# schreibfaul1/ESP32-Opus-Player

Hardware: AMD Instinct MI355X
Metric: decoded 48 kHz stereo frames/sec/GPU (x real-time); HBM GB/s vs roofline (higher is better)
Workload: dtype int32 fixed-point (int16/int32 with 64-bit products); 1 GPU; celt_fb_stereo_64k; streams_per_gpu=65536

## Files before the change

### __graft_entry__.py

```python
import importlib.util
import os
import subprocess
import sys

ROOT = os.path.dirname(os.path.abspath(__file__))
PKG_DIR = os.path.join(ROOT, "esp32-opus-player_amd")
CSRC = os.path.join(PKG_DIR, "csrc")


def _load_pkg():
    name = "esp32_opus_player_amd"
    if name in sys.modules:
        return sys.modules[name]
    path = os.path.join(PKG_DIR, "__init__.py")
    spec = importlib.util.spec_from_file_location(name, path, submodule_search_locations=[PKG_DIR])
    mod = importlib.util.module_from_spec(spec)
    sys.modules[name] = mod
    spec.loader.exec_module(mod)
    return mod


def build() -> None:
    subprocess.check_call([sys.executable, os.path.join(ROOT, "tools", "gen_rom_tables.py")])
    hipcc = os.environ.get("HIPCC", "/opt/rocm/bin/hipcc")
    out = os.path.join(PKG_DIR, "libopusgpu.so")
    cmd = [hipcc, "--offload-arch=gfx950", "-O3", "-std=c++17", "-fPIC", "-shared",
           os.path.join(CSRC, "og_api.hip"), os.path.join(CSRC, "og_recon.hip"), os.path.join(CSRC, "og_parse64.hip"), os.path.join(CSRC, "og_rfc.hip"), os.path.join(CSRC, "og_silk_nb.hip"), os.path.join(CSRC, "og_silk_synth.hip"), os.path.join(CSRC, "og_compat.cpp"),
           os.path.join(CSRC, "og_pages.cpp"), os.path.join(CSRC, "og_files.cpp"),
           "-I", os.path.join(ROOT, "include"), "-pthread",
           "-o", out]
    cmd = [c for c in cmd if not c.endswith("og_compat.cpp") or os.path.exists(c)]
    flags_file = os.path.join(CSRC, "BUILD_FLAGS")
    if os.path.exists(flags_file):
        cmd += open(flags_file).read().split()
    subprocess.check_call(cmd)
    subprocess.check_call(["make", "-C", os.path.join(ROOT, "oracle"), "-s"])
    emul = os.path.join(ROOT, "tests", "emul")
    if os.path.exists(os.path.join(emul, "Makefile")):
        subprocess.check_call(["make", "-C", emul, "-s"])
    pkg = _load_pkg()
    lib = pkg.load_lib()
    missing = [s for s in pkg.EXPORTS if not hasattr(lib, s)]
    if missing:
        raise RuntimeError(f"libopusgpu.so lacks exports: {missing}")


def smoke() -> None:
    import numpy as np
    sys.path.insert(0, os.path.join(ROOT, "tests"))
    import oracle_py
    pkg = _load_pkg()
    oracle = oracle_py.load()
    ctx = pkg.Context(0)
    n, frames = 64, 3
    for name, toc, L in (("CELT-FB", pkg.TOC_CELT_FB_STEREO, 160), ("SILK-NB", pkg.TOC_SILK_NB_STEREO, 40),
                         ("hybrid FB", pkg.TOC_HYBRID_FB_STEREO, 120)):
        pay = pkg.lcg_payloads(n, frames, L)
        ref, ok = oracle.batch_decode(2, toc, pay)
        assert ok == n * frames
        ctx.streams_alloc(n, 2)
        for f in range(frames):
            pk = [bytes([toc]) + pay[f, s].tobytes() for s in range(n)]
            pcm, res = ctx.decode_packets(np.arange(n), pk)
            assert (res == 960).all(), (name, res)
            assert (pcm == ref[:, f]).all(), f"{name}: GPU PCM differs from the oracle"
    ctx.close()
    print("smoke ok: 64 streams x 3 frames x {CELT-FB, SILK-NB, hybrid FB} bit-exact vs oracle")


if __name__ == "__main__":
    build()
    if len(sys.argv) > 1 and sys.argv[1] == "smoke":
        smoke()
```

### esp32-opus-player_amd/csrc/og_api.hip

```cpp
#include <hip/hip_runtime.h>
#include <stdio.h>
#include <stdlib.h>
#include <string.h>
#include <condition_variable>
#include <functional>
#include <memory>
#include <new>
#include <mutex>
#include <thread>
#include <vector>
#include "og_decode.hpp"
#include "og_host_framing.hpp"
#include "og_output.hpp"
#include "og_debug.hpp"

using namespace og;

static_assert(sizeof(opusgpu_frame_desc) == sizeof(FrameDesc), "descriptor layout");

#define OG_STALL_MAX_SPINS (1 << 20)
__global__ void __launch_bounds__(64) k_stream_stall(long long ticks, int max_spins) {
    const long long t0 = wall_clock64();
    for (int i = 0; i < max_spins && wall_clock64() - t0 < ticks; i++) __builtin_amdgcn_s_sleep(8);
}
__global__ void __launch_bounds__(64) k_stream_init(StreamState *st, int first, int count, int channels, int full) {
    const int s = first + (int)blockIdx.x;
    if ((int)blockIdx.x >= count) return;
    if (full)
        stream_init(&st[s], channels);
    else
        stream_reset(&st[s]);
}

enum {
    CRC_CHUNK = 64,
    CRC_DEPTH = 1,
    CRC_LPL = CRC_CHUNK / 16,
    CRC_PPI = 64 / CRC_LPL,
    CRC_NL = 64 / CRC_PPI,
    CRC_ROW = CRC_CHUNK / 4 + 1,
    CRC_STEPS = CRC_CHUNK / 8
};
__global__ void __launch_bounds__(256) k_pages_crc(const u8 *__restrict__ blob, const long long *__restrict__ offs,
                                                    const i32 *__restrict__ lens, i32 *__restrict__ status, int n,
                                                    const u32 *__restrict__ tables) {
    __shared__ u32 T[8][256];
    __shared__ u32 tile[4][64 * CRC_ROW];
    __shared__ long long pg_start[4][64];
    __shared__ i32 pg_meta[4][64];
    for (int i = (int)threadIdx.x; i < 8 * 256; i += 256) T[i >> 8][i & 255] = tables[i];
    const int wv = (int)threadIdx.x >> 6, lane = (int)threadIdx.x & 63;
    const int p = (int)blockIdx.x * 256 + (int)threadIdx.x;
    int total = 0, st = OPUSGPU_PAGE_BAD_CAPTURE;
    u32 want = 0;
    long long at0 = 0;
    if (p < n) {
        const u8 *pg = blob + offs[p];
        const int len = lens[p];
        if (len >= 27) {
            u32 h[8];
            if (len >= 32) {
                const uint4 a = *reinterpret_cast<const uint4 *>(pg), b = *reinterpret_cast<const uint4 *>(pg + 16);
                h[0] = a.x; h[1] = a.y; h[2] = a.z; h[3] = a.w; h[4] = b.x; h[5] = b.y; h[6] = b.z; h[7] = b.w;
            } else {
                for (int i = 0; i < 8; i++) h[i] = 0;
                for (int i = 0; i < 27; i++) h[i >> 2] |= (u32)pg[i] << (8 * (i & 3));
            }
            const int nseg = (int)(h[6] >> 16) & 255, hdr = 27 + nseg;
            if (h[0] == 0x5367674fu  && (h[1] & 255u) == 0 && len >= hdr) {
                u32 body = 0;
                for (int i = 0; i < nseg; i += 16) {
                    u32 v[4];
                    if (27 + i + 16 <= len) {
                        const uint4 q = *reinterpret_cast<const uint4 *>(pg + 27 + i);
                        v[0] = q.x; v[1] = q.y; v[2] = q.z; v[3] = q.w;
                    } else {
                        v[0] = v[1] = v[2] = v[3] = 0;
                        for (int b = 0; b < 16 && i + b < nseg; b++) v[b >> 2] |= (u32)pg[27 + i + b] << (8 * (b & 3));
                    }
                    const int keep = nseg - i;
#pragma unroll
                    for (int d = 0; d < 4; d++) {
                        const int kd = keep - 4 * d;
                        const u32 m = kd >= 4 ? 0xffffffffu : kd <= 0 ? 0u : (1u << (8 * kd)) - 1u;
                        body = __builtin_amdgcn_sad_u8(v[d] & m, 0u, body);
                    }
                }
                if (len >= hdr + (int)body) {
                    total = hdr + (int)body;
                    st = 0;
                    want = h[5] >> 16 | h[6] << 16;
                }
            }
        }
        at0 = offs[p];
    }
    const int z = st < 0 ? 0 : (int)((reinterpret_cast<unsigned long long>(blob) + (unsigned long long)at0) & (unsigned long long)(CRC_CHUNK - 1));
    const int nfull = (z + total) / CRC_CHUNK, tail = (z + total) % CRC_CHUNK, chunks = nfull + (tail != 0);
    pg_start[wv][lane] = at0 - z;
    pg_meta[wv][lane] = z | total << 8;
    __syncthreads();
    int max_chunks = chunks;
    for (int d = 32; d; d >>= 1) max_chunks = max(max_chunks, __shfl_xor(max_chunks, d, 64));
    u32 crc = 0;
    const int grp = lane / CRC_LPL, quarter = lane % CRC_LPL;
    auto fetch = [&](int k, u32 (&w)[CRC_NL][4]) {
#pragma unroll
        for (int i = 0; i < CRC_NL; i++) {
            const int q = CRC_PPI * i + grp;
            const i32 meta = pg_meta[wv][q];
            const int idx = CRC_CHUNK * k + 16 * quarter - (meta & 255);
            w[i][0] = w[i][1] = w[i][2] = w[i][3] = 0u;
            if (idx > -16 && idx < (meta >> 8)) {
                const uint4 v = *reinterpret_cast<const uint4 *>(
                    __builtin_assume_aligned(blob + (pg_start[wv][q] + CRC_CHUNK * k + 16 * quarter), 16));
                w[i][0] = v.x; w[i][1] = v.y; w[i][2] = v.z; w[i][3] = v.w;
                if (idx < 26) {
#pragma unroll
                    for (int d = 0; d < 4; d++) {
                        u32 m = 0;
#pragma unroll
                        for (int c = 0; c < 4; c++) {
                            const int ib = idx + 4 * d + c;
                            if (ib >= 0 && !(ib >= 22 && ib <= 25)) m |= 0xffu << (8 * c);
                        }
                        w[i][d] &= m;
                    }
                }
            }
        }
    };
    auto consume = [&](int k, u32 (&w)[CRC_NL][4]) {
#pragma unroll
        for (int i = 0; i < CRC_NL; i++) {
            u32 *dst = &tile[wv][(CRC_PPI * i + grp) * CRC_ROW + 4 * quarter];
            dst[0] = w[i][0]; dst[1] = w[i][1]; dst[2] = w[i][2]; dst[3] = w[i][3];
        }
        __builtin_amdgcn_fence(__ATOMIC_RELEASE, "wavefront");
        __builtin_amdgcn_wave_barrier();
        __builtin_amdgcn_fence(__ATOMIC_ACQUIRE, "wavefront");
        if (k + CRC_DEPTH < max_chunks) fetch(k + CRC_DEPTH, w);
        const u32 *rowp = &tile[wv][lane * CRC_ROW];
        const int steps = k < nfull ? CRC_STEPS : k == nfull ? tail >> 3 : 0;
#pragma unroll
        for (int j = 0; j < CRC_STEPS; j++) {
            if (j < steps) {
                const u32 lo = rowp[2 * j], hi = rowp[2 * j + 1];
                const u32 a = crc ^ ((lo & 0xffu) << 24 | (lo & 0xff00u) << 8 | (lo >> 8 & 0xff00u) | lo >> 24);
                crc = T[7][a >> 24] ^ T[6][(a >> 16) & 255] ^ T[5][(a >> 8) & 255] ^ T[4][a & 255] ^ T[3][hi & 255] ^
                      T[2][(hi >> 8) & 255] ^ T[1][(hi >> 16) & 255] ^ T[0][hi >> 24];
            }
        }
        if (k == nfull && (tail & 7)) {
            const int base = tail & ~7;
            for (int b = 0; b < (tail & 7); b++) {
                const int i = base + b;
                crc = crc << 8 ^ T[0][crc >> 24 ^ (rowp[i >> 2] >> (8 * (i & 3)) & 255u)];
            }
        }
        __builtin_amdgcn_fence(__ATOMIC_RELEASE, "wavefront");
        __builtin_amdgcn_wave_barrier();
        __builtin_amdgcn_fence(__ATOMIC_ACQUIRE, "wavefront");
    };
    u32 wa[CRC_NL][4], wb[CRC_NL][4];
    if (max_chunks > 0) fetch(0, wa);
    if (CRC_DEPTH == 2) {
        if (max_chunks > 1) fetch(1, wb);
        for (int k = 0; k < max_chunks; k += 2) {
            consume(k, wa);
            if (k + 1 < max_chunks) consume(k + 1, wb);
        }
    } else {
        for (int k = 0; k < max_chunks; k++) consume(k, wa);
    }
    if (p < n) status[p] = st < 0 ? st : (i32)(crc == want);
}

static_assert(sizeof(opusgpu_output_cfg) == sizeof(OutputCfg) && sizeof(OutputCfg) == 4, "output cfg layout");
__global__ void __launch_bounds__(256) k_output_stage(const i16 *__restrict__ pcm, long long pcm_stride, const i32 *__restrict__ valid_of,
                                                       int valid_all, int block_samples, const OutputCfg *__restrict__ cfg_of,
                                                       OutputCfg cfg_all, u32 *__restrict__ out, long long out_stride,
                                                       int units_per_block, long long n_units, int vec_ok) {
    const long long t = (long long)blockIdx.x * 256 + threadIdx.x;
    if (t >= n_units) return;
    const int b = (int)(t / units_per_block), w0 = 4 * (int)(t - (long long)b * units_per_block);
    const OutputCfg c = cfg_of ? cfg_of[b] : cfg_all;
    int valid = valid_of ? valid_of[b] : valid_all;
    valid = valid > block_samples ? block_samples : valid;
    const int count = output_words(c, valid);
    if (w0 >= count) return;
    const i16 *blk = pcm + (size_t)b * pcm_stride;
    u32 *dst = out + (size_t)b * out_stride + w0;
    if (vec_ok && c.bits == 16 && c.channels == 2 && w0 + 4 <= count) {
        const uint4 v = *reinterpret_cast<const uint4 *>(blk + 2 * w0);
        const u32 in[4] = {v.x, v.y, v.z, v.w};
        u32 o[4];
#pragma unroll
        for (int j = 0; j < 4; j++) {
            i32 l = (i32)(i16)(in[j] & 0xffffu), r = (i32)(i16)(in[j] >> 16);
            if (c.force_mono) l = r = (i32)(i16)((l + r) / 2);
            o[j] = output_pack(l, r, false, (i32)c.volume);
        }
        *reinterpret_cast<uint4 *>(dst) = make_uint4(o[0], o[1], o[2], o[3]);
    } else {
        for (int j = 0; j < 4 && w0 + j < count; j++) dst[j] = output_word(blk, w0 + j, c);
    }
}

#ifndef OG_WAVES_PER_SIMD
#define OG_WAVES_PER_SIMD 1
#endif
#define OG_RECON_WAVES 2
#define OG_SILK_WAVES 2
__global__ void __launch_bounds__(64, OG_WAVES_PER_SIMD) k_decode_step(const FrameDesc *__restrict__ descs, const u8 *__restrict__ arena,
                                                   StreamState *st, i16 *pcm, i32 *result, int n, int n_streams,
                                                   int pcm_stride, int skip_celt, SilkHandoff *handoff, const SilkRec *srecs,
                                                   int q4_only) {
    unsigned long long todo = 1ull;
    int base = (int)blockIdx.x;
    if (q4_only) {
        base = (int)blockIdx.x * 64;
        const int f0 = base + (int)threadIdx.x;
        bool mine = false;
        if (f0 < n) {
            const FrameDesc d0 = descs[f0];
            mine = d0.stream >= 0 && d0.stream < n_streams && !desc_rfc(d0.flags) && desc_mode(d0.flags) == MODE_SILK && handoff[f0].valid == 2;
        }
        todo = __ballot(mine);
    }
    while (todo) {
        const int f = base + (int)__builtin_ctzll(todo);
        todo &= todo - 1;
        if (f >= n) return;
        const FrameDesc d = descs[f];
        int ret;
        if (d.stream < 0 || d.stream >= n_streams) {
            ret = BAD_ARG;
        } else if (desc_rfc(d.flags)) {
            continue;
        } else if (skip_celt && desc_mode(d.flags) == MODE_CELT) {
            continue;
        } else {
            StreamState *s = &st[d.stream];
#ifdef OG_PROF_SINGLE
            OG_PROF_INIT();
#endif
            ret = decode_frame_wave<true>(s, arena + d.offset, d.len, desc_mode(d.flags), desc_bandwidth(d.flags),
                                          desc_channels(d.flags), pcm + (size_t)f * pcm_stride, handoff ? &handoff[f] : nullptr,
                                          srecs ? &srecs[f] : nullptr, q4_only, desc_mode_after(d.flags));
#ifdef OG_PROF_SINGLE
            OG_PROF_FLUSH();
#endif
            if (ret == CONTINUE_SPLIT) continue;
        }
        if (threadIdx.x == 0) result[f] = ret;
        __syncthreads();
    }
}

extern "C" void og_launch_silk_synth(hipStream_t s, const void *descs, const void *arena, void *streams, void *pcm, void *result, int n,
                                     int n_streams, int pcm_stride, void *handoff, const void *srecs, int nb_elsewhere);
extern "C" void og_launch_silk_synth_nb(hipStream_t s, const void *descs, const void *arena, void *streams, void *pcm, void *result, int n,
                                        int n_streams, int pcm_stride, void *handoff, const void *srecs, int nb_elsewhere);

#define OG_SPARSE_WAVES 4
template <int LANES>
OG_DEV void silk_parse_kernel_body(const FrameDesc *__restrict__ descs, const u8 *__restrict__ arena, const StreamState *st, SilkRec *srecs,
                                   SilkHandoff *handoff, int n, int n_streams, SilkShadow *shadow, u32 epoch) {
    silk_tables_load();
    if ((int)threadIdx.x >= LANES) return;
    const int f = (int)blockIdx.x * LANES + (int)threadIdx.x;
    if (f >= n) return;
    const FrameDesc d = descs[f];
    const int mode = desc_mode(d.flags);
    if (d.stream < 0 || d.stream >= n_streams || mode == MODE_CELT || desc_rfc(d.flags)) return;
#ifdef OG_PROF_SPARSE
    OG_PROF_INIT();
#endif
    SilkShadow *const sh = shadow ? &shadow[d.stream] : nullptr;
    const SilkPast past(&st[d.stream], sh, epoch);
    silk_parse_lane(past, arena + d.offset, d.len, mode, desc_bandwidth(d.flags), desc_channels(d.flags), &srecs[f], &handoff[f], sh, epoch,
                    desc_mode_after(d.flags));
#ifdef OG_PROF_SPARSE
    OG_PROF_FLUSH();
#endif
}
__global__ void __launch_bounds__(64, OG_SPARSE_WAVES) k_silk_parse(const FrameDesc *__restrict__ descs, const u8 *__restrict__ arena,
                                                      const StreamState *st, SilkRec *srecs, SilkHandoff *handoff, int n,
                                                      int n_streams, SilkShadow *shadow, u32 epoch) {
    silk_parse_kernel_body<32>(descs, arena, st, srecs, handoff, n, n_streams, shadow, epoch);
}
__global__ void __launch_bounds__(64, OG_SPARSE_WAVES) k_silk_parse64(const FrameDesc *__restrict__ descs, const u8 *__restrict__ arena,
                                                        const StreamState *st, SilkRec *srecs, SilkHandoff *handoff, int n,
                                                        int n_streams, SilkShadow *shadow, u32 epoch) {
    silk_parse_kernel_body<64>(descs, arena, st, srecs, handoff, n, n_streams, shadow, epoch);
}

#define OG_SPARAMS_WAVES 4
__global__ void __launch_bounds__(64, OG_SPARAMS_WAVES) k_silk_params(const FrameDesc *__restrict__ descs, const StreamState *st, SilkRec *srecs,
                                                                       int n, int n_streams, SilkShadow *shadow, u32 epoch) {
    constexpr int FR = OG_PAR_LANES / 2;
    const int ch = (int)threadIdx.x / FR, f = (int)blockIdx.x * FR + (int)threadIdx.x % FR;
    bool act = f < n;
    FrameDesc d = {0, 0, 0, 0};
    if (act) {
        d = descs[f];
        act = !(d.stream < 0 || d.stream >= n_streams || desc_mode(d.flags) == MODE_CELT || desc_rfc(d.flags));
    }
    SilkShadow *const sh = act && shadow ? &shadow[d.stream] : nullptr;
    const SilkParPast past(act ? &st[d.stream] : st, sh, epoch);
    const int mode = desc_mode(d.flags), channels = desc_channels(d.flags);
    SilkParTask t;
    t.skip = 1;
    if (act) silk_params_channel(past, mode, desc_bandwidth(d.flags), channels, &srecs[f], ch, t);
    OG_FULL_SYNC();
    if (act) silk_params_shadow(past, t, channels, &srecs[f], ch, sh, epoch);
}

#define OG_PARSE_KERNEL_NAME k_celt_parse
#include "og_parse_kernel.hpp"
extern "C" void og_launch_celt_parse64(hipStream_t s, int grid, const void *descs, const void *arena, void *streams, void *recs, int n,
                                       int n_streams, const void *handoff, int which, int groups, unsigned *started);
extern "C" int og_celt_parse64_frames(void);

extern "C" void og_launch_celt_recon_fb(hipStream_t s, const void *descs, void *streams, const void *recs, void *rout, int n,
                                        int n_streams, int hybrid, unsigned *started);
extern "C" int og_celt_recon_fb_signals(int n);
extern "C" void og_launch_decode_rfc(hipStream_t s, const void *descs, const void *arena, void *streams, void *pcm, void *result, int n,
                                     int n_streams, int pcm_stride);
__global__ void __launch_bounds__(64, OG_RECON_WAVES) k_celt_recon(const FrameDesc *__restrict__ descs, StreamState *st,
                                                                      const ParseRec *recs, ReconOut *rout, int n,
                                                                      int n_streams, int hybrid, int rest_only) {
    unsigned long long todo = 1ull;
    int base = (int)blockIdx.x;
    if (rest_only) {
        base = (int)blockIdx.x * 64;
        const int f0 = base + (int)threadIdx.x;
        bool mine = false;
        if (f0 < n) {
            const FrameDesc d0 = descs[f0];
            const int m0 = desc_mode(d0.flags);
            if (d0.stream >= 0 && d0.stream < n_streams && (m0 == MODE_CELT || (m0 == MODE_HYBRID && hybrid)) && !desc_rfc(d0.flags)) {
                const u32 fl = recs[f0].flags;
                const bool fast = !(fl & (RF_SKIP | RF_BAD_CELT)) && ((fl >> RF_LM_SHIFT) & 3) == 3 && recs[f0].n_words < REC_MAX_WORDS &&
                                  recs[f0].n_leaves <= FAST_MAX_LEAVES;
                mine = !fast && !(m0 == MODE_HYBRID && (fl & RF_SKIP));
            }
        }
        todo = __ballot(mine);
    }
    while (todo) {
        const int f = base + (int)__builtin_ctzll(todo);
        todo &= todo - 1;
        if (f >= n) return;
        const FrameDesc d = descs[f];
        const int mode = desc_mode(d.flags);
        if (d.stream < 0 || d.stream >= n_streams || !(mode == MODE_CELT || (mode == MODE_HYBRID && hybrid)) || desc_rfc(d.flags)) continue;
        if (mode == MODE_HYBRID && (recs[f].flags & RF_SKIP)) continue;
#if !defined(OG_PROF_PARSE) && !defined(OG_PROF_SINGLE) && !defined(OG_PROF_SPARSE) && !defined(OG_PROF_SSYNTH)
        OG_PROF_INIT();
#endif
        const int pos = OG_UNI(st[d.stream].celt.ring_pos);
        const int ret = celt_recon_wave(&st[d.stream], &recs[f], mode, desc_channels(d.flags), rest_only ? RECON_REST_ONLY : RECON_ALL, desc_mode_after(d.flags));
        if (ret != RECON_NOT_MINE && threadIdx.x == 0) rout[f] = ReconOut{ret, pos};
#if !defined(OG_PROF_PARSE) && !defined(OG_PROF_SINGLE) && !defined(OG_PROF_SPARSE) && !defined(OG_PROF_SSYNTH)
        OG_PROF_FLUSH();
#endif
        __syncthreads();
    }
}

static __device__ __forceinline__ i32 pk_add_sat_i16(i32 a, i32 b) {
    typedef short s2 __attribute__((ext_vector_type(2)));
    const s2 r = __builtin_elementwise_add_sat(__builtin_bit_cast(s2, a), __builtin_bit_cast(s2, b));
    return __builtin_bit_cast(i32, r);
}
__global__ void __launch_bounds__(64) k_celt_post(const FrameDesc *__restrict__ descs, StreamState *st, const ParseRec *recs,
                                                  const ReconOut *__restrict__ rout, i32 *__restrict__ result, i16 *pcm, int n,
                                                  int n_streams, int channels, int pcm_stride, const SilkHandoff *handoff,
                                                  int modes, int others_ran) {
    struct RowInfo {
        const i32 *ring;
        i16 *pcm;
        const i16 *silk;
        int pos, silk_n;
    };
    constexpr int CS = 32, PCS = CS / 4, RSTEP = 64 / PCS;
    __shared__ RowInfo rows[64];
    __shared__ __attribute__((aligned(16))) i32 tin[64][CS + 4];
    __shared__ __attribute__((aligned(16))) i16 tout[64][CS + 8];
    const int lane = (int)threadIdx.x;
    const int t = (int)blockIdx.x * 64 + lane;
    const int f = channels == 2 ? t >> 1 : t, c = channels == 2 ? t & 1 : 0;
    bool live = false, emit = false;
    StreamState *ss = nullptr;
    const i16 *silk = nullptr;
    int silk_n = 0;
    int pos = 0;
    if (f < n) {
        const FrameDesc d = descs[f];
        const int mode = desc_mode(d.flags);
        const bool stream_ok = d.stream >= 0 && d.stream < n_streams;
        if (!(modes >> (d.flags & 3) & 1) || (!stream_ok && !others_ran)) {
            if (c == 0) result[f] = BAD_ARG;
        } else if (stream_ok && (mode == MODE_CELT || (mode == MODE_HYBRID && handoff)) && !desc_rfc(d.flags)) {
            const u32 rf = recs[f].flags;
            if (!(mode == MODE_HYBRID && (rf & RF_SKIP))) {
                const ReconOut ro = rout[f];
                if (c == 0) result[f] = ro.ret;
                if (!(rf & (RF_SKIP | RF_BAD_CELT))) {
                    live = true;
                    ss = &st[d.stream];
                    emit = ro.ret >= 0;
                    pos = ro.pos & RING_MASK;
                    if (mode == MODE_HYBRID) {
                        silk = handoff[f].pcm;
                        silk_n = 960 * desc_channels(d.flags);
                    }
                }
            }
        }
    }
    i16 *out = pcm + (size_t)(f < n ? f : 0) * pcm_stride;
    const bool fast = channels == 2 && __all(live && emit && (pos & (CS - 1)) == 0);
    if (!fast) {
        if (live) celt_post_lane(&ss->celt, c, channels, 960, pos, emit ? out : nullptr, silk, silk_n);
        return;
    }
    rows[lane].ring = ss->celt.ring[c];
    rows[lane].pcm = out;
    rows[lane].silk = silk;
    rows[lane].pos = pos;
    rows[lane].silk_n = silk_n;
    __syncthreads();
    const int q = lane % PCS, r0 = lane / PCS;
    const i32 *src[PCS];
    int spos[PCS];
#pragma unroll
    for (int k = 0; k < PCS; k++) {
        src[k] = rows[r0 + RSTEP * k].ring;
        spos[k] = rows[r0 + RSTEP * k].pos + 4 * q;
    }
    og_v4i v[PCS];
#pragma unroll
    for (int k = 0; k < PCS; k++) v[k] = *reinterpret_cast<const og_v4i *>(src[k] + (spos[k] & RING_MASK));
    i32 m = ss->celt.deemph[c];
    for (int ch = 0; ch < 960 / CS; ch++) {
#pragma unroll
        for (int k = 0; k < PCS; k++) *reinterpret_cast<og_v4i *>(&tin[r0 + RSTEP * k][4 * q]) = v[k];
        if (ch + 1 < 960 / CS) {
#pragma unroll
            for (int k = 0; k < PCS; k++) v[k] = *reinterpret_cast<const og_v4i *>(src[k] + ((spos[k] + CS * (ch + 1)) & RING_MASK));
        }
        __syncthreads();
#pragma unroll
        for (int g8 = 0; g8 < CS / 8; g8++) {
            i16 o[8];
#pragma unroll
            for (int h = 0; h < 2; h++) {
                const og_v4i sv = *reinterpret_cast<const og_v4i *>(&tin[lane][8 * g8 + 4 * h]);
                i32 tt = sv.x + m;
                m = mul16x32_q15(27853, tt);
                o[4 * h + 0] = (i16)sat16(pshr32(tt, 12));
                tt = sv.y + m;
                m = mul16x32_q15(27853, tt);
                o[4 * h + 1] = (i16)sat16(pshr32(tt, 12));
                tt = sv.z + m;
                m = mul16x32_q15(27853, tt);
                o[4 * h + 2] = (i16)sat16(pshr32(tt, 12));
                tt = sv.w + m;
                m = mul16x32_q15(27853, tt);
                o[4 * h + 3] = (i16)sat16(pshr32(tt, 12));
            }
            og_v4i w;
            w.x = (i32)((u32)(u16)o[0] | (u32)(u16)o[1] << 16);
            w.y = (i32)((u32)(u16)o[2] | (u32)(u16)o[3] << 16);
            w.z = (i32)((u32)(u16)o[4] | (u32)(u16)o[5] << 16);
            w.w = (i32)((u32)(u16)o[6] | (u32)(u16)o[7] << 16);
            *reinterpret_cast<og_v4i *>(&tout[lane][8 * g8]) = w;
        }
        __syncthreads();
#pragma unroll
        for (int k = 0; k < PCS / 2; k++) {
            const int fr = r0 + RSTEP * k;
            const og_v2u L = *reinterpret_cast<const og_v2u *>(&tout[2 * fr][4 * q]);
            const og_v2u R = *reinterpret_cast<const og_v2u *>(&tout[2 * fr + 1][4 * q]);
            og_v4i w;
            w.x = (i32)((L.x & 0xffffu) | R.x << 16);
            w.y = (i32)(L.x >> 16 | (R.x & 0xffff0000u));
            w.z = (i32)((L.y & 0xffffu) | R.y << 16);
            w.w = (i32)(L.y >> 16 | (R.y & 0xffff0000u));
            const int at = (CS * ch + 4 * q) * 2;
            const i16 *const sk = rows[2 * fr].silk;
            if (sk && at < rows[2 * fr].silk_n) {
                const og_v4i a = *reinterpret_cast<const og_v4i *>(sk + at);
                w.x = pk_add_sat_i16(w.x, a.x);
                w.y = pk_add_sat_i16(w.y, a.y);
                w.z = pk_add_sat_i16(w.z, a.z);
                w.w = pk_add_sat_i16(w.w, a.w);
            }
            *reinterpret_cast<og_v4i *>(rows[2 * fr].pcm + at) = w;
        }
    }
    ss->celt.deemph[c] = m;
}

#include "og_step.hpp"

const size_t og_parse_rec_bytes = sizeof(ParseRec), og_recon_out_bytes = sizeof(ReconOut), og_silk_handoff_bytes = sizeof(SilkHandoff),
             og_silk_rec_bytes = sizeof(SilkRec);
namespace {
struct StepRange {
    const FrameDesc *dd;
    i16 *pp;
    i32 *rr;
    ParseRec *recs;
    ReconOut *rout;
    SilkHandoff *hh;
    SilkRec *srecs;
    StepRange(const Step &st, size_t f0)
        : dd((const FrameDesc *)st.descs + f0), pp((i16 *)st.pcm + f0 * (size_t)st.pcm_stride), rr((i32 *)st.result + f0),
          recs((ParseRec *)st.recs + f0), rout((ReconOut *)st.rout + f0), hh(st.handoff ? (SilkHandoff *)st.handoff + f0 : nullptr),
          srecs(st.srecs ? (SilkRec *)st.srecs + f0 : nullptr) {}
};
}
void launch_stream_stall(opusgpu_ctx *ctx, hipStream_t q) {
    hipLaunchKernelGGL(k_stream_stall, dim3(1), dim3(64), 0, q, ctx->stall_ticks, (int)OG_STALL_MAX_SPINS);
}
void launch_decode_rfc(opusgpu_ctx *ctx, hipStream_t q, const Step &st) {
    og_launch_decode_rfc(q, st.descs, st.arena, ctx->d_streams, st.pcm, st.result, st.n, ctx->n_streams, st.pcm_stride);
}
void launch_decode_step(opusgpu_ctx *ctx, hipStream_t q, const Step &st, size_t f0, int cnt, int pass) {
    const StepRange r(st, f0);
    hipLaunchKernelGGL(k_decode_step, dim3(pass == 2 ? (cnt + 63) / 64 : cnt), dim3(64), 0, q, r.dd, (const u8 *)st.arena, ctx->d_streams, r.pp,
                       r.rr, cnt, ctx->n_streams, st.pcm_stride, pass ? 1 : 0, pass == 2 ? r.hh : nullptr,
                       (const SilkRec *)(pass == 2 ? r.srecs : nullptr), pass == 2 ? 1 : 0);
}
void launch_silk_parse(opusgpu_ctx *ctx, hipStream_t q, const Step &st, size_t f0, int cnt, void *shadow, uint32_t epoch) {
    const StepRange r(st, f0);
    hipLaunchKernelGGL(k_silk_parse, dim3((cnt + 31) / 32), dim3(64), 0, q, r.dd, (const u8 *)st.arena, (const StreamState *)ctx->d_streams,
                       r.srecs, r.hh, cnt, ctx->n_streams, (SilkShadow *)shadow, epoch);
}
void launch_silk_parse64(opusgpu_ctx *ctx, hipStream_t q, const Step &st, size_t f0, int cnt, void *shadow, uint32_t epoch) {
    const StepRange r(st, f0);
    hipLaunchKernelGGL(k_silk_parse64, dim3((cnt + 63) / 64), dim3(64), 0, q, r.dd, (const u8 *)st.arena, (const StreamState *)ctx->d_streams,
                       r.srecs, r.hh, cnt, ctx->n_streams, (SilkShadow *)shadow, epoch);
}
void launch_silk_params(opusgpu_ctx *ctx, hipStream_t q, const Step &st, size_t f0, int cnt, void *shadow, uint32_t epoch) {
    const StepRange r(st, f0);
    hipLaunchKernelGGL(k_silk_params, dim3((cnt + OG_PAR_LANES / 2 - 1) / (OG_PAR_LANES / 2)), dim3(64), 0, q, r.dd,
                       (const StreamState *)ctx->d_streams, r.srecs, cnt, ctx->n_streams, (SilkShadow *)shadow, epoch);
}
int celt_parse_early_grid(const opusgpu_ctx *ctx, int cnt, bool wide) {
    const int per = (wide ? og_celt_parse64_frames() : OG_PL_FRAMES) * ctx->parse_groups;
    return (cnt + per - 1) / per;
}
void launch_celt_parse(opusgpu_ctx *ctx, hipStream_t q, const Step &st, size_t f0, int cnt, bool wide, bool early) {
    const StepRange r(st, f0);
    const int which = early ? (int)PARSE_CELT_ONLY : (int)PARSE_ALL, groups = early ? ctx->parse_groups : 1;
    const int per = wide ? og_celt_parse64_frames() : OG_PL_FRAMES;
    const int grid = early ? celt_parse_early_grid(ctx, cnt, wide) : (cnt + per - 1) / per;
    u32 *const started = early ? ctx->sp.d_started : nullptr;
    if (wide)
        og_launch_celt_parse64(q, grid, r.dd, st.arena, ctx->d_streams, r.recs, cnt, ctx->n_streams, r.hh, which, groups, started);
    else
        hipLaunchKernelGGL(k_celt_parse, dim3(grid), dim3(64 * OG_PL_WAVES), 0, q, r.dd, (const u8 *)st.arena, ctx->d_streams, r.recs, cnt,
                           ctx->n_streams, (const SilkHandoff *)r.hh, which, groups, started);
}
void launch_celt_recon_fb(opusgpu_ctx *ctx, hipStream_t q, const Step &st, size_t f0, int cnt, bool counts_in) {
    const StepRange r(st, f0);
    og_launch_celt_recon_fb(q, r.dd, ctx->d_streams, r.recs, r.rout, cnt, ctx->n_streams, r.hh ? 1 : 0, counts_in ? ctx->sp.d_started + 16 : nullptr);
}
void launch_celt_recon(opusgpu_ctx *ctx, hipStream_t q, const Step &st, size_t f0, int cnt) {
    const StepRange r(st, f0);
    hipLaunchKernelGGL(k_celt_recon, dim3(ctx->fast_recon ? (cnt + 63) / 64 : cnt), dim3(64), 0, q, r.dd, ctx->d_streams, (const ParseRec *)r.recs,
                       r.rout, cnt, ctx->n_streams, r.hh ? 1 : 0, ctx->fast_recon);
}
void launch_celt_post(opusgpu_ctx *ctx, hipStream_t q, const Step &st, size_t f0, int cnt, bool others) {
    const StepRange r(st, f0);
    hipLaunchKernelGGL(k_celt_post, dim3((cnt * ctx->channels + 63) / 64), dim3(64), 0, q, r.dd, ctx->d_streams, (const ParseRec *)r.recs,
                       (const ReconOut *)r.rout, r.rr, r.pp, cnt, ctx->n_streams, ctx->channels, st.pcm_stride, (const SilkHandoff *)r.hh, st.modes,
                       others ? 1 : 0);
}
void launch_silk_synth(opusgpu_ctx *ctx, hipStream_t q, const Step &st, size_t f0, int cnt, int nb_done) {
    const StepRange r(st, f0);
    og_launch_silk_synth(q, r.dd, st.arena, ctx->d_streams, r.pp, r.rr, cnt, ctx->n_streams, st.pcm_stride, r.hh, r.srecs, nb_done);
}
void launch_silk_synth_nb(opusgpu_ctx *ctx, hipStream_t q, const Step &st, size_t f0, int cnt) {
    const StepRange r(st, f0);
    og_launch_silk_synth_nb(q, r.dd, st.arena, ctx->d_streams, r.pp, r.rr, cnt, ctx->n_streams, st.pcm_stride, r.hh, r.srecs, 1);
}


extern "C" {


int opusgpu_version(void) { return 100; }

int opusgpu_ctx_create(int device, opusgpu_ctx **out) {
    if (!out || device < 0) return OPUSGPU_BAD_ARG;
    *out = nullptr;
    int count = 0;
    if (hipGetDeviceCount(&count) != hipSuccess || count <= 0 || device >= count) return OPUSGPU_ERR_NO_DEVICE;
    if (hipSetDevice(device) != hipSuccess) return OPUSGPU_ERR_NO_DEVICE;
    hipFuncAttributes attr;
    if (hipFuncGetAttributes(&attr, reinterpret_cast<const void *>(k_decode_step)) != hipSuccess) {
        (void)hipGetLastError();
        return OPUSGPU_ERR_NO_DEVICE;
    }
    opusgpu_ctx *ctx = new (std::nothrow) opusgpu_ctx();
    if (!ctx) return OPUSGPU_ALLOC_FAIL;
    ctx->device = device;
    ctx->split_celt = og_debug().split;
    ctx->split_hybrid = og_debug().split_hybrid;
    ctx->fast_recon = og_debug().fast_recon;
    ctx->parse_groups = og_debug().parse_groups;
    ctx->host_parts = og_debug().host_parts;
    if (og_debug().stall_us) {
        int khz = 0;
        if (hipDeviceGetAttribute(&khz, hipDeviceAttributeWallClockRate, device) != hipSuccess || khz <= 0) {
            (void)hipGetLastError();
            delete ctx;
            return OPUSGPU_ERR_HIP;
        }
        ctx->stall_ticks = (long long)og_debug().stall_us * khz / 1000;
    }
    if (hipStreamCreateWithFlags(&ctx->stream, hipStreamNonBlocking) != hipSuccess) {
        delete ctx;
        return OPUSGPU_ERR_HIP;
    }
    *out = ctx;
    return OPUSGPU_OK;
}

void opusgpu_ctx_destroy(opusgpu_ctx *ctx) {
    if (!ctx) return;
    (void)hipSetDevice(ctx->device);
    (void)hipStreamSynchronize(ctx->stream);
    (void)hipFree(ctx->d_streams);
    (void)hipFree(ctx->d_descs);
    (void)hipFree(ctx->d_arena);
    (void)hipFree(ctx->d_pcm);
    (void)hipFree(ctx->d_result);
    pipeline_destroy(ctx);
    for (int i = 0; i < 6; i++) {
        (void)hipFree(ctx->d_recs[i]);
        (void)hipFree(ctx->d_rout[i]);
    }
    for (int i = 0; i < OG_SILK_SETS; i++) {
        (void)hipFree(ctx->d_handoff[i]);
        (void)hipFree(ctx->d_srecs[i]);
    }
    (void)hipFree(ctx->d_shadow);
    (void)hipHostFree(ctx->h_pcm);
    (void)hipHostFree(ctx->h_res);
    (void)hipHostFree(ctx->h_arena);
    (void)hipHostFree(ctx->h_descs);
    (void)hipFree(ctx->d_crc_tables);
    for (hipEvent_t e : ctx->ev_piece)
        if (e) (void)hipEventDestroy(e);
    for (hipEvent_t e : ctx->ev_part)
        if (e) (void)hipEventDestroy(e);
    if (ctx->copy_stream) (void)hipStreamDestroy(ctx->copy_stream);
    (void)hipStreamDestroy(ctx->stream);
    delete ctx;
}

const char *opusgpu_last_error(const opusgpu_ctx *ctx) { return ctx ? ctx->err : "no context"; }
int opusgpu_set_mode(opusgpu_ctx *ctx, int mode) {
    if (!ctx || (mode != OPUSGPU_MODE_REFERENCE && mode != OPUSGPU_MODE_RFC)) return OPUSGPU_BAD_ARG;
    ctx->mode = mode;
    return OPUSGPU_OK;
}
int opusgpu_get_mode(const opusgpu_ctx *ctx) { return ctx ? ctx->mode : OPUSGPU_MODE_REFERENCE; }
int opusgpu_set_pipeline(opusgpu_ctx *ctx, int on) {
    if (!ctx) return OPUSGPU_BAD_ARG;
    HIPCHK(ctx, hipSetDevice(ctx->device));
    if (on)
        if (int rc = pipeline_create(ctx)) return rc;
    if ((on != 0) != (ctx->pipeline != 0)) {
        HIPCHK(ctx, hipDeviceSynchronize());
        ctx->sp.drained();
        ctx->sp.last_kind = 0;
        ctx->sp.shadow_epoch++;
    }
    ctx->pipeline = on ? 1 : 0;
    return OPUSGPU_OK;
}
int opusgpu_get_pipeline(const opusgpu_ctx *ctx) { return ctx ? ctx->pipeline : 0; }
size_t opusgpu_stream_state_bytes(void) { return sizeof(StreamState); }
int opusgpu_stream_count(const opusgpu_ctx *ctx) { return ctx ? ctx->n_streams : 0; }
int opusgpu_stream_channels(const opusgpu_ctx *ctx) { return ctx ? ctx->channels : 0; }

int opusgpu_streams_reset(opusgpu_ctx *ctx, int first, int count, int full) {
    if (!ctx || first < 0 || count < 0 || first + count > ctx->n_streams) return OPUSGPU_BAD_ARG;
    if (count == 0) return OPUSGPU_OK;
    HIPCHK(ctx, hipSetDevice(ctx->device));
    if (int rc = sync_in_flight(ctx)) return rc;
    ctx->sp.drained();
    ctx->sp.shadow_epoch++;
    hipLaunchKernelGGL(k_stream_init, dim3(count), dim3(64), 0, ctx->stream, ctx->d_streams, first, count, ctx->channels,
                       full ? 1 : 0);
    HIPCHK(ctx, hipGetLastError());
    HIPCHK(ctx, hipStreamSynchronize(ctx->stream));
    for (int i = first; i < first + count; i++) ctx->last_count[i] = ctx->last_flags[i] = 0;
    return OPUSGPU_OK;
}

int opusgpu_streams_alloc(opusgpu_ctx *ctx, int n_streams, int channels) {
    if (!ctx || n_streams <= 0 || (channels != 1 && channels != 2)) return OPUSGPU_BAD_ARG;
    HIPCHK(ctx, hipSetDevice(ctx->device));
    HIPCHK(ctx, hipStreamSynchronize(ctx->stream));
    if (int rc = sync_in_flight(ctx)) return rc;
    if (ctx->d_streams) {
        HIPCHK(ctx, hipFree(ctx->d_streams));
        ctx->d_streams = nullptr;
        ctx->n_streams = 0;
    }
    hipError_t e = hipMalloc((void **)&ctx->d_streams, sizeof(StreamState) * (size_t)n_streams);
    if (e != hipSuccess) return fail(ctx, OPUSGPU_ALLOC_FAIL, "hipMalloc(streams)", e);
    if (ctx->d_shadow) HIPCHK(ctx, hipFree(ctx->d_shadow));
    ctx->d_shadow = nullptr;
    e = hipMalloc(&ctx->d_shadow, sizeof(SilkShadow) * (size_t)n_streams);
    if (e != hipSuccess) return fail(ctx, OPUSGPU_ALLOC_FAIL, "hipMalloc(shadow)", e);
    HIPCHK(ctx, hipMemset(ctx->d_shadow, 0, sizeof(SilkShadow) * (size_t)n_streams));
    ctx->sp.shadow_epoch++;
    ctx->n_streams = n_streams;
    ctx->channels = channels;
    ctx->last_count.assign((size_t)n_streams, 0);
    ctx->last_flags.assign((size_t)n_streams, 0);
    return opusgpu_streams_reset(ctx, 0, n_streams, 1);
}

int opusgpu_dev_alloc(opusgpu_ctx *ctx, size_t bytes, void **dptr) {
    if (!ctx || !dptr) return OPUSGPU_BAD_ARG;
    HIPCHK(ctx, hipSetDevice(ctx->device));
    if (bytes > SIZE_MAX - 16) return OPUSGPU_ALLOC_FAIL;
    hipError_t e = hipMalloc(dptr, bytes + 16);
    if (e != hipSuccess) return fail(ctx, OPUSGPU_ALLOC_FAIL, "hipMalloc", e);
    return OPUSGPU_OK;
}
int opusgpu_dev_free(opusgpu_ctx *ctx, void *dptr) {
    if (!ctx) return OPUSGPU_BAD_ARG;
    HIPCHK(ctx, hipSetDevice(ctx->device));
    HIPCHK(ctx, hipFree(dptr));
    return OPUSGPU_OK;
}
int opusgpu_memcpy_h2d(opusgpu_ctx *ctx, void *dst, const void *src, size_t bytes) {
    if (!ctx) return OPUSGPU_BAD_ARG;
    HIPCHK(ctx, hipSetDevice(ctx->device));
    HIPCHK(ctx, hipMemcpyAsync(dst, src, bytes, hipMemcpyHostToDevice, ctx->stream));
    HIPCHK(ctx, hipStreamSynchronize(ctx->stream));
    return OPUSGPU_OK;
}
int opusgpu_memcpy_d2h(opusgpu_ctx *ctx, void *dst, const void *src, size_t bytes) {
    if (!ctx) return OPUSGPU_BAD_ARG;
    HIPCHK(ctx, hipSetDevice(ctx->device));
    if (int rc = sync_in_flight(ctx)) return rc;
    HIPCHK(ctx, hipMemcpyAsync(dst, src, bytes, hipMemcpyDeviceToHost, ctx->stream));
    HIPCHK(ctx, hipStreamSynchronize(ctx->stream));
    return OPUSGPU_OK;
}


int opusgpu_decode_step_device(opusgpu_ctx *ctx, int n, const void *d_descs, const void *d_arena, void *d_pcm,
                               void *d_result, void *hip_stream) {
    return decode_step_impl(ctx, n, d_descs, d_arena, d_pcm, d_result, hip_stream, true);
}
int opusgpu_decode_step_device_modes(opusgpu_ctx *ctx, int n, const void *d_descs, const void *d_arena, void *d_pcm,
                                     void *d_result, void *hip_stream, int modes) {
    if (modes <= 0 || modes > 15 || (modes & 7) == 0) return OPUSGPU_BAD_ARG;
    return decode_step_impl(ctx, n, d_descs, d_arena, d_pcm, d_result, hip_stream, true, modes);
}
int opusgpu_decode_steps_device(opusgpu_ctx *ctx, int n_steps, const int32_t *n, const void *const *d_descs, const void *const *d_arena,
                                void *const *d_pcm, void *const *d_result, void *hip_stream, int modes) {
    if (!ctx || n_steps < 0 || modes < 0 || modes > 7) return OPUSGPU_BAD_ARG;
    if (n_steps == 0) return OPUSGPU_OK;
    if (!n || !d_descs || !d_arena || !d_pcm || !d_result) return OPUSGPU_BAD_ARG;
    if (!ctx->d_streams) return OPUSGPU_BAD_ARG;
    int max_n = 0;
    for (int k = 0; k < n_steps; k++) {
        if (n[k] < 0) return OPUSGPU_BAD_ARG;
        if (n[k] > 0 && (!d_descs[k] || !d_arena[k] || ((uintptr_t)d_arena[k] & 15) || !d_pcm[k] || !d_result[k])) return OPUSGPU_BAD_ARG;
        max_n = OG_MAX(max_n, n[k]);
    }
    if (max_n == 0) return OPUSGPU_OK;
    return decode_window(ctx, n_steps, n, max_n, d_descs, d_arena, d_pcm, d_result, hip_stream, modes ? modes : 7);
}

#ifdef OG_PROF
extern "C" int og_recon_fb_prof(unsigned long long *out64, int reset);
extern "C" int og_rfc_prof(unsigned long long *out64, int reset);
extern "C" int og_ssynth_prof(unsigned long long *out64, int reset);
extern "C" int og_ssynth_nb_prof(unsigned long long *out64, int reset);
int opusgpu_debug_prof(unsigned long long *out64, int reset) {
    unsigned long long fb[64], rf[64];
    if (og_recon_fb_prof(fb, reset) != 0 || og_rfc_prof(rf, reset) != 0) return -1;
    for (int i = 0; i < 64; i++) fb[i] += rf[i];
    if (og_ssynth_prof(rf, reset) != 0) return -1;
    for (int i = 0; i < 64; i++) fb[i] += rf[i];
    if (og_ssynth_nb_prof(rf, reset) != 0) return -1;
    for (int i = 0; i < 64; i++) fb[i] += rf[i];
    if (hipMemcpyFromSymbol(out64, HIP_SYMBOL(g_prof), sizeof(unsigned long long) * 64) != hipSuccess) return -1;
    for (int i = 0; i < 64; i++) out64[i] += fb[i];
    if (reset) {
        unsigned long long z[64] = {0};
        if (hipMemcpyToSymbol(HIP_SYMBOL(g_prof), z, sizeof(z)) != hipSuccess) return -1;
    }
    return 0;
}
#endif

int opusgpu_pages_crc_device(opusgpu_ctx *ctx, int n_pages, const void *d_blob, const void *d_offsets, const void *d_lens,
                             void *d_status, void *hip_stream) {
    if (!ctx || n_pages < 0) return OPUSGPU_BAD_ARG;
    if (n_pages == 0) return OPUSGPU_OK;
    if (!d_blob || !d_offsets || !d_lens || !d_status) return OPUSGPU_BAD_ARG;
    HIPCHK(ctx, hipSetDevice(ctx->device));
    hipStream_t s = hip_stream ? (hipStream_t)hip_stream : ctx->stream;
    if (!ctx->d_crc_tables) {
        static u32 t[8][256];
        for (u32 i = 0; i < 256; i++) {
            u32 r = i << 24;
            for (int k = 0; k < 8; k++) r = (r & 0x80000000u) ? (r << 1) ^ 0x04c11db7u : r << 1;
            t[0][i] = r;
        }
        for (int j = 1; j < 8; j++)
            for (u32 i = 0; i < 256; i++) t[j][i] = (t[j - 1][i] << 8) ^ t[0][t[j - 1][i] >> 24];
        if (hipMalloc((void **)&ctx->d_crc_tables, sizeof(t)) != hipSuccess) return OPUSGPU_ALLOC_FAIL;
        HIPCHK(ctx, hipMemcpy(ctx->d_crc_tables, t, sizeof(t), hipMemcpyHostToDevice));
    }
    hipLaunchKernelGGL(k_pages_crc, dim3((n_pages + 255) / 256), dim3(256), 0, s, (const u8 *)d_blob, (const long long *)d_offsets,
                       (const i32 *)d_lens, (i32 *)d_status, n_pages, (const u32 *)ctx->d_crc_tables);
    HIPCHK(ctx, hipGetLastError());
    return OPUSGPU_OK;
}

int opusgpu_output_stage_device(opusgpu_ctx *ctx, int n_blocks, int block_samples, const void *d_pcm, long long pcm_stride,
                                const void *d_valid, int valid_all, const void *d_cfgs, opusgpu_output_cfg cfg, void *d_i2s,
                                long long i2s_stride, void *hip_stream) {
    if (!ctx || n_blocks < 0 || block_samples < 0) return OPUSGPU_BAD_ARG;
    if (n_blocks == 0 || block_samples == 0) return OPUSGPU_OK;
    if (!d_pcm || !d_i2s || pcm_stride < 0 || i2s_stride < 0) return OPUSGPU_BAD_ARG;
    if (!d_valid && (valid_all < 0 || valid_all > block_samples)) return OPUSGPU_BAD_ARG;
    if (!d_cfgs && ((cfg.bits != 8 && cfg.bits != 16) || (cfg.channels != 1 && cfg.channels != 2))) return OPUSGPU_BAD_ARG;
    HIPCHK(ctx, hipSetDevice(ctx->device));
    hipStream_t s = hip_stream ? (hipStream_t)hip_stream : ctx->stream;
    const int max_words = (d_cfgs || (cfg.bits == 8 && cfg.channels == 1)) ? 2 * block_samples : block_samples;
    const int units = (max_words + 3) / 4;
    const long long n_units = (long long)units * n_blocks;
    const int vec_ok = ((uintptr_t)d_pcm % 16 == 0 && pcm_stride % 8 == 0 && (uintptr_t)d_i2s % 16 == 0 && i2s_stride % 4 == 0) ? 1 : 0;
    OutputCfg c;
    memcpy(&c, &cfg, sizeof c);
    hipLaunchKernelGGL(k_output_stage, dim3((unsigned)((n_units + 255) / 256)), dim3(256), 0, s, (const i16 *)d_pcm, pcm_stride,
                       (const i32 *)d_valid, valid_all, block_samples, (const OutputCfg *)d_cfgs, c, (u32 *)d_i2s, i2s_stride, units,
                       n_units, vec_ok);
    HIPCHK(ctx, hipGetLastError());
    return OPUSGPU_OK;
}

int opusgpu_synchronize(opusgpu_ctx *ctx) {
    if (!ctx) return OPUSGPU_BAD_ARG;
    HIPCHK(ctx, hipStreamSynchronize(ctx->stream));
    return OPUSGPU_OK;
}

int opusgpu_event_create(opusgpu_ctx *ctx, void **event) {
    if (!ctx || !event) return OPUSGPU_BAD_ARG;
    hipEvent_t e;
    HIPCHK(ctx, hipEventCreate(&e));
    *event = (void *)e;
    return OPUSGPU_OK;
}
int opusgpu_event_record(opusgpu_ctx *ctx, void *event) {
    if (!ctx || !event) return OPUSGPU_BAD_ARG;
    HIPCHK(ctx, hipEventRecord((hipEvent_t)event, ctx->stream));
    return OPUSGPU_OK;
}
int opusgpu_event_elapsed_ms(opusgpu_ctx *ctx, void *start, void *stop, float *ms) {
    if (!ctx || !start || !stop || !ms) return OPUSGPU_BAD_ARG;
    HIPCHK(ctx, hipEventSynchronize((hipEvent_t)stop));
    HIPCHK(ctx, hipEventElapsedTime(ms, (hipEvent_t)start, (hipEvent_t)stop));
    return OPUSGPU_OK;
}
int opusgpu_event_destroy(opusgpu_ctx *ctx, void *event) {
    if (!ctx || !event) return OPUSGPU_BAD_ARG;
    HIPCHK(ctx, hipEventDestroy((hipEvent_t)event));
    return OPUSGPU_OK;
}

static std::mutex g_copy_stream_mutex;
static int copy_stream_of(opusgpu_ctx *ctx, hipStream_t *out) {
    std::lock_guard<std::mutex> lock(g_copy_stream_mutex);
    if (!ctx->copy_stream) HIPCHK(ctx, hipStreamCreateWithFlags(&ctx->copy_stream, hipStreamNonBlocking));
    *out = ctx->copy_stream;
    return OPUSGPU_OK;
}
int opusgpu_upload_async(opusgpu_ctx *ctx, void *dst, const void *src, size_t bytes) {
    if (!ctx || (bytes && (!dst || !src))) return OPUSGPU_BAD_ARG;
    HIPCHK(ctx, hipSetDevice(ctx->device));
    hipStream_t cs;
    if (int rc = copy_stream_of(ctx, &cs)) return rc;
    if (bytes) HIPCHK(ctx, hipMemcpyAsync(dst, src, bytes, hipMemcpyHostToDevice, cs));
    return OPUSGPU_OK;
}
int opusgpu_upload_fence(opusgpu_ctx *ctx, void *event) {
    if (!ctx || !event) return OPUSGPU_BAD_ARG;
    HIPCHK(ctx, hipSetDevice(ctx->device));
    hipStream_t cs;
    if (int rc = copy_stream_of(ctx, &cs)) return rc;
    HIPCHK(ctx, hipEventRecord((hipEvent_t)event, cs));
    return OPUSGPU_OK;
}
int opusgpu_stream_wait_event(opusgpu_ctx *ctx, void *event, void *hip_stream) {
    if (!ctx || !event) return OPUSGPU_BAD_ARG;
    HIPCHK(ctx, hipSetDevice(ctx->device));
    HIPCHK(ctx, hipStreamWaitEvent(hip_stream ? (hipStream_t)hip_stream : ctx->stream, (hipEvent_t)event, 0));
    if ((!hip_stream || (hipStream_t)hip_stream == ctx->stream) && ctx->sp.parse_stream) {
        HIPCHK(ctx, hipStreamWaitEvent(ctx->sp.parse_stream, (hipEvent_t)event, 0));
        HIPCHK(ctx, hipStreamWaitEvent(ctx->sp.recon_stream, (hipEvent_t)event, 0));
    }
    return OPUSGPU_OK;
}
int opusgpu_event_synchronize(opusgpu_ctx *ctx, void *event) {
    if (!ctx || !event) return OPUSGPU_BAD_ARG;
    HIPCHK(ctx, hipSetDevice(ctx->device));
    HIPCHK(ctx, hipEventSynchronize((hipEvent_t)event));
    return OPUSGPU_OK;
}
int opusgpu_host_register(opusgpu_ctx *ctx, void *ptr, size_t bytes) {
    if (!ctx || !ptr || !bytes) return OPUSGPU_BAD_ARG;
    HIPCHK(ctx, hipSetDevice(ctx->device));
    hipError_t e = hipHostRegister(ptr, bytes, hipHostRegisterDefault);
    if (e != hipSuccess) return fail(ctx, OPUSGPU_ALLOC_FAIL, "hipHostRegister", e);
    std::lock_guard<std::mutex> lock(ctx->registered_mutex);
    ctx->registered.emplace_back((uintptr_t)ptr, bytes);
    return OPUSGPU_OK;
}
int opusgpu_host_unregister(opusgpu_ctx *ctx, void *ptr) {
    if (!ctx || !ptr) return OPUSGPU_BAD_ARG;
    HIPCHK(ctx, hipSetDevice(ctx->device));
    {
        std::lock_guard<std::mutex> lock(ctx->registered_mutex);
        for (size_t i = 0; i < ctx->registered.size(); i++)
            if (ctx->registered[i].first == (uintptr_t)ptr) {
                ctx->registered.erase(ctx->registered.begin() + i);
                break;
            }
    }
    HIPCHK(ctx, hipHostUnregister(ptr));
    return OPUSGPU_OK;
}

int opusgpu_stream_state_get(opusgpu_ctx *ctx, int index, void *dst, size_t bytes) {
    if (!ctx || !dst || index < 0 || index >= ctx->n_streams || bytes > sizeof(StreamState)) return OPUSGPU_BAD_ARG;
    return opusgpu_memcpy_d2h(ctx, dst, &ctx->d_streams[index], bytes);
}

int opusgpu_stream_pitch_get(opusgpu_ctx *ctx, int index, int32_t out[4]) {
    if (!ctx || !out || index < 0 || index >= ctx->n_streams) return OPUSGPU_BAD_ARG;
    int32_t head[2], ch0[3];
    if (int rc = opusgpu_memcpy_d2h(ctx, head, &ctx->d_streams[index], sizeof(head))) return rc;
    const SilkChannel *c = &ctx->d_streams[index].silk.ch[0];
    HIPCHK(ctx, hipMemcpy(&ch0[0], &c->prevSignalType, 4, hipMemcpyDeviceToHost));
    HIPCHK(ctx, hipMemcpy(&ch0[1], &c->lagPrev, 4, hipMemcpyDeviceToHost));
    HIPCHK(ctx, hipMemcpy(&ch0[2], &c->fs_kHz, 4, hipMemcpyDeviceToHost));
    out[0] = head[1];
    out[1] = ch0[0];
    out[2] = ch0[1];
    out[3] = ch0[2];
    return OPUSGPU_OK;
}

int opusgpu_debug_stage_taps(opusgpu_ctx *ctx, int slot, opusgpu_stage_taps *out) {
    if (!ctx || !out || slot < 0 || slot >= ctx->last_n || !ctx->last_descs) return OPUSGPU_BAD_ARG;
    HIPCHK(ctx, hipSetDevice(ctx->device));
    if (int rc = sync_in_flight(ctx)) return rc;
    HIPCHK(ctx, hipStreamSynchronize(ctx->stream));
    memset(out, 0, sizeof(*out));
    FrameDesc d;
    HIPCHK(ctx, hipMemcpy(&d, (const FrameDesc *)ctx->last_descs + slot, sizeof(d), hipMemcpyDeviceToHost));
    if (d.stream < 0 || d.stream >= ctx->n_streams) return OPUSGPU_BAD_ARG;
    const int mode = MODE_SILK + (d.flags & 3);
    std::unique_ptr<StreamState> st(new (std::nothrow) StreamState);
    if (!st) return OPUSGPU_ALLOC_FAIL;
    HIPCHK(ctx, hipMemcpy(st.get(), &ctx->d_streams[d.stream], sizeof(StreamState), hipMemcpyDeviceToHost));
    if (mode != MODE_SILK && ctx->last_recs) {
        std::unique_ptr<ParseRec> r(new (std::nothrow) ParseRec);
        if (!r) return OPUSGPU_ALLOC_FAIL;
        HIPCHK(ctx, hipMemcpy(r.get(), (const ParseRec *)ctx->last_recs + slot, sizeof(ParseRec), hipMemcpyDeviceToHost));
        out->celt_valid = 1;
        out->celt_ret = r->ret;
        out->silence = (r->flags & RF_SILENCE) != 0;
        out->transient = (r->flags & RF_TRANSIENT) != 0;
        out->lm = (int)(r->flags >> RF_LM_SHIFT) & 3;
        out->spread = (int)(r->flags >> RF_SPREAD_SHIFT) & 3;
        out->dual_stereo = (r->flags & RF_DUAL) != 0;
        out->anti_collapse_on = (r->flags & RF_ANTI_COLLAPSE) != 0;
        out->intensity = r->intensity;
        out->pf_pitch = r->pf_pitch;
        out->pf_gain = r->pf_gain;
        out->pf_tapset = r->pf_tapset;
        out->n_leaves = r->n_leaves;
        out->celt_rng_final = r->rng_final;
        memcpy(out->bandE, r->bandE, sizeof(out->bandE));
        memcpy(out->pulses, r->pulses, sizeof(out->pulses));
        memcpy(out->tf_res, r->tf_res, sizeof(out->tf_res));
    }
    const CeltState &c = st->celt;
    for (int ch = 0; ch < 2; ch++) {
        for (int i = 0; i < 960; i++) out->syn_post[ch][i] = c.ring[ch][(c.ring_pos - 960 + i) & RING_MASK];
        for (int i = 0; i < 60; i++) out->overlap_tail[ch][i] = c.tail[ch][i];
    }
    memcpy(out->state_bandE, c.bandE, sizeof(out->state_bandE));
    memcpy(out->state_logE1, c.logE1, sizeof(out->state_logE1));
    memcpy(out->state_logE2, c.logE2, sizeof(out->state_logE2));
    out->state_rng = c.rng;
    out->pf_period = c.pf_period;
    out->pf_gain_state = c.pf_gain;
    out->pf_tapset_state = c.pf_tapset;
    if (mode != MODE_CELT && ctx->last_had_silk_recs && ctx->last_srecs) {
        std::unique_ptr<SilkRec> r(new (std::nothrow) SilkRec);
        if (!r) return OPUSGPU_ALLOC_FAIL;
        HIPCHK(ctx, hipMemcpy(r.get(), (const SilkRec *)ctx->last_srecs + slot, sizeof(SilkRec), hipMemcpyDeviceToHost));
        out->silk_valid = 1;
        out->silk_ret = r->ret;
        out->decode_only_middle = r->decode_only_middle;
        out->ms_pred_q13[0] = r->MS_pred_Q13[0];
        out->ms_pred_q13[1] = r->MS_pred_Q13[1];
        for (int ch = 0; ch < 2; ch++) {
            const SilkRecCh &k = r->ch[ch];
            memcpy(out->silk_ch[ch].pitchL, k.pitchL, sizeof(k.pitchL));
            memcpy(out->silk_ch[ch].Gains_Q16, k.Gains_Q16, sizeof(k.Gains_Q16));
            memcpy(out->silk_ch[ch].PredCoef_Q12, k.PredCoef_Q12, sizeof(k.PredCoef_Q12));
            memcpy(out->silk_ch[ch].LTPCoef_Q14, k.LTPCoef_Q14, sizeof(k.LTPCoef_Q14));
            out->silk_ch[ch].LTP_scale_Q14 = k.LTP_scale_Q14;
            out->silk_ch[ch].signalType = k.signalType;
            out->silk_ch[ch].quantOffsetType = k.quantOffsetType;
        }
    }
    for (int ch = 0; ch < 2; ch++) {
        memcpy(out->silk_out[ch], st->silk.ch[ch].outBuf, sizeof(out->silk_out[ch]));
        memcpy(out->silk_sLPC_Q14[ch], st->silk.ch[ch].sLPC_Q14_buf, sizeof(out->silk_sLPC_Q14[ch]));
        out->silk_fs_kHz[ch] = st->silk.ch[ch].fs_kHz;
    }
    return OPUSGPU_OK;
}

int opusgpu_packet_to_frames(const uint8_t *packet, int32_t len, int32_t stream, opusgpu_frame_desc descs[48]) {
    return opusgpu_packet_to_frames_mode(packet, len, stream, OPUSGPU_MODE_REFERENCE, descs);
}

int opusgpu_packet_to_frames_mode(const uint8_t *packet, int32_t len, int32_t stream, int mode, opusgpu_frame_desc descs[48]) {
    if (!packet || !descs) return OPUSGPU_BAD_ARG;
    if (len <= 0) return len == 0 ? OPUSGPU_INVALID_PACKET : OPUSGPU_BAD_ARG;
    return ogh::packet_to_frames_mode(packet, len, stream, mode, descs);
}

int opusgpu_empty_packet_to_frames(int32_t stream, int32_t last_flags, int decoder_channels, int frame_size, opusgpu_frame_desc descs[48]) {
    if (!descs || frame_size <= 0 || frame_size % 120 || (decoder_channels != 1 && decoder_channels != 2)) return OPUSGPU_BAD_ARG;
    const int count = (frame_size + OPUSGPU_FRAME_SAMPLES - 1) / OPUSGPU_FRAME_SAMPLES;
    if (count > 48) return OPUSGPU_BAD_ARG;
    const int32_t flags = ogh::empty_flags(last_flags, decoder_channels);
    for (int i = 0; i < count; i++) descs[i] = opusgpu_frame_desc{stream, 0, 0, flags};
    return count;
}

static int grow(opusgpu_ctx *ctx, void **p, size_t *cap, size_t need) {
    if (*cap >= need) return OPUSGPU_OK;
    if (*p) HIPCHK(ctx, hipFree(*p));
    *p = nullptr;
    *cap = 0;
    size_t want = need + need / 2 + 256;
    hipError_t e = hipMalloc(p, want);
    if (e != hipSuccess) return fail(ctx, OPUSGPU_ALLOC_FAIL, "hipMalloc(staging)", e);
    *cap = want;
    return OPUSGPU_OK;
}

}

#include "og_host_path.hpp"

#include "og_ms.hpp"
#include "og_files_run.hpp"
#include "og_tracks.hpp"
#include "og_ms_tracks.hpp"
```

### esp32-opus-player_amd/csrc/og_celt_rec.hpp

```cpp
#pragma once
#include <stddef.h>
#include "og_state.hpp"

namespace og {

constexpr int REC_BAND_WORDS = 4;
constexpr int REC_MAX_LEAVES = NBANDS * 2 * 16;
constexpr int REC_MAX_WORDS = NBANDS * (REC_BAND_WORDS + 2 * 33) + 3 * NBANDS + 1;

enum {
    RF_SILENCE = 1, RF_TRANSIENT = 2, RF_LM_SHIFT = 2 , RF_STEREO = 16, RF_SPREAD_SHIFT = 5 ,
    RF_DUAL = 128, RF_ANTI_COLLAPSE = 256, RF_RC_ERROR = 512, RF_TELL_OVERFLOW = 1024,
    RF_SKIP = 2048,
    RF_BAD_CELT = 4096
};
enum {
    BW_SIGN0 = 1, BW_SIGN1 = 2, BW_INV = 4, BW_SIGN = 8, BW_MID_FIRST = 16, BW_SWAP = 32,
    BW_THETA0 = 64, BW_THETA1 = 128,
    BW_TF_SHIFT = 8 , BW_FOLD0_SHIFT = 11 , BW_FOLD1_SHIFT = 16 ,
    BW_HAS_LOW = 1 << 21, BW_DUAL = 1 << 22, BW_DUAL_END = 1 << 23, BW_STEREO = 1 << 24,
    BW_DUAL_PRE = 1 << 25
};
enum {
    JW_NPVQ_SHIFT = 5 , JW_FIRST_SHIFT = 10 , JW_NEED_LOW = 1 << 20,
    LW_OFF_SHIFT = 8 , LW_B_SHIFT = 12 , LW_N_SHIFT = 16
};

struct SilkHandoff {
    alignas(128) i16 pcm[1920];
    u32 valid;
    u32 storage, end_offs, end_window;
    i32 nend_bits, nbits_total;
    u32 offs, rng, val, ext;
    i32 rem, error;
};
static_assert(sizeof(SilkHandoff) % 128 == 0 && offsetof(SilkHandoff, pcm) == 0, "handoff alignment");

struct ParseRec {
    i32 ret;
    u32 rng_final;
    u32 flags;
    i32 intensity, pf_pitch, pf_gain, pf_tapset, start;
    i32 n_leaves, n_words;
    u32 need_norm;
    i32 n_coef;
    i32 reserved[4];
    i16 bandE[2 * NBANDS];
    i16 pulses[NBANDS];
    u16 band_w[NBANDS];
    i8 tf_res[NBANDS];
    i8 pad[256 - 64 - 4 * NBANDS - 2 * NBANDS - 2 * NBANDS - NBANDS];
    struct Leaf {
        u32 idx;
        u32 geom;
        u32 aux;
        u32 pad;
    } leaf[REC_MAX_LEAVES];
    u32 words[(REC_MAX_WORDS + 64) / 64 * 64];
    i32 work_pulses[NBANDS];
    i32 work_pad[32 - NBANDS];
};
static_assert(offsetof(ParseRec, leaf) % 16 == 0 && offsetof(ParseRec, words) % 16 == 0 && offsetof(ParseRec, work_pulses) % 16 == 0 &&
              offsetof(ParseRec, work_pad) == offsetof(ParseRec, work_pulses) + 4 * NBANDS && NBANDS + 3 <= 32, "16-byte stores into the record");
static_assert(sizeof(ParseRec) % 16 == 0, "record alignment");

constexpr int FAST_MAX_LEAVES = 416;

struct ReconOut {
    i32 ret, pos;
};

}
```

### esp32-opus-player_amd/csrc/og_celt_recon.hpp

```cpp
#pragma once
#include "og_celt.hpp"
#include "og_celt_rec.hpp"

namespace og {

#ifdef OG_HOST_EMUL
OG_DEV i32 rot_dot2(u32 pair, u32 coef, i32 half) {
    return (i32)((u32)mul16((i32)pair, (i32)coef) + (u32)mul16((i32)(pair >> 16), (i32)(coef >> 16)) + (u32)half) >> 15;
}
OG_DEV u32 rot_pack(i32 lo, i32 hi) { return ((u32)lo & 0xffffu) | (u32)hi << 16; }
#else
OG_DEV i32 rot_dot2(u32 pair, u32 coef, i32 half) {
    i32 r;
    asm("v_dot2_i32_i16 %0, %1, %2, %3" : "=v"(r) : "v"(pair), "v"(coef), "v"(half));
    return r >> 15;
}
OG_DEV u32 rot_pack(i32 lo, i32 hi) { return __builtin_amdgcn_perm((u32)hi, (u32)lo, 0x05040100u); }
#endif
OG_DEV void rotate_chain(i16 *const p0, int r, int len, int stride, u32 k_a, u32 k_b) {
    const i32 half = 16384;
    int i = r, steps = 0;
    i32 x1 = p0[i];
    for (; i + 3 * stride < len - stride; i += 4 * stride, steps += 4) {
        const i32 e1 = p0[i + stride], e2 = p0[i + 2 * stride], e3 = p0[i + 3 * stride], e4 = p0[i + 4 * stride];
        u32 pk = rot_pack(x1, e1);
        const i32 o0 = rot_dot2(pk, k_a, half);
        x1 = rot_dot2(pk, k_b, half);
        pk = rot_pack(x1, e2);
        const i32 o1 = rot_dot2(pk, k_a, half);
        x1 = rot_dot2(pk, k_b, half);
        pk = rot_pack(x1, e3);
        const i32 o2 = rot_dot2(pk, k_a, half);
        x1 = rot_dot2(pk, k_b, half);
        pk = rot_pack(x1, e4);
        const i32 o3 = rot_dot2(pk, k_a, half);
        x1 = rot_dot2(pk, k_b, half);
        p0[i] = (i16)o0;
        p0[i + stride] = (i16)o1;
        p0[i + 2 * stride] = (i16)o2;
        p0[i + 3 * stride] = (i16)o3;
    }
    for (; i < len - stride; i += stride, steps++) {
        const u32 pk = rot_pack(x1, p0[i + stride]);
        p0[i] = (i16)rot_dot2(pk, k_a, half);
        x1 = rot_dot2(pk, k_b, half);
    }
    p0[i] = (i16)x1;
    if (steps >= 2) {
        i -= 2 * stride;
        i32 x2 = p0[i + stride];
        for (; i - 3 * stride >= 0; i -= 4 * stride) {
            const i32 e1 = p0[i], e2 = p0[i - stride], e3 = p0[i - 2 * stride], e4 = p0[i - 3 * stride];
            u32 pk = rot_pack(e1, x2);
            const i32 o0 = rot_dot2(pk, k_b, half);
            x2 = rot_dot2(pk, k_a, half);
            pk = rot_pack(e2, x2);
            const i32 o1 = rot_dot2(pk, k_b, half);
            x2 = rot_dot2(pk, k_a, half);
            pk = rot_pack(e3, x2);
            const i32 o2 = rot_dot2(pk, k_b, half);
            x2 = rot_dot2(pk, k_a, half);
            pk = rot_pack(e4, x2);
            const i32 o3 = rot_dot2(pk, k_b, half);
            x2 = rot_dot2(pk, k_a, half);
            p0[i + stride] = (i16)o0;
            p0[i] = (i16)o1;
            p0[i - stride] = (i16)o2;
            p0[i - 2 * stride] = (i16)o3;
        }
        for (; i >= 0; i -= stride) {
            const u32 pk = rot_pack(p0[i], x2);
            p0[i + stride] = (i16)rot_dot2(pk, k_b, half);
            x2 = rot_dot2(pk, k_a, half);
        }
        p0[r] = (i16)x2;
    }
}
OG_DEV void rotate1_lane(i16 *xv, int x, int len, int stride, i32 c, i32 s) {
    const u32 k_a = rot_pack(c, -s), k_b = rot_pack(s, c);
    for (int r = 0; r < stride; r++) {
        if (r >= len - stride) break;
        rotate_chain(xv + x, r, len, stride, k_a, k_b);
    }
}

struct RotJob {
    int x, blen, logB, stride2;
    i32 c, s;
    bool on;
};
#ifndef OG_HOST_EMUL
OG_DEV void pvq_rotate_wave(i16 *xv, const RotJob &j, u8 *marker) {
    if (!__any(j.on)) return;
    const int lane = OG_LANE;
    const int w_geo = j.x | j.blen << 16, w_par = j.logB | j.stride2 << 8;
    const int w_cs = (int)((u32)(u16)j.c | (u32)(u16)j.s << 16);
    for (int pass = 0; pass < 2; pass++) {
        int chains = 0;
        if (j.on) chains = pass == 0 ? (j.stride2 ? OG_MAX(0, OG_MIN(j.stride2, j.blen - j.stride2)) : 0) : (j.blen >= 2);
        const int cnt = chains << j.logB;
        const int incl = wave_scan_add(cnt), excl = incl - cnt;
        const int total = __builtin_amdgcn_readlane(incl, 63);
        for (int base = 0; base < total; base += 64) {
            marker[lane] = 0;
            OG_LSYNC();
            if (cnt > 0 && excl < base + 64 && incl > base) marker[OG_MAX(excl - base, 0)] = (u8)(lane + 1);
            OG_LSYNC();
            const int leaf = wave_scan_max((int)marker[lane]) - 1;
            const int item = base + lane;
            const bool work = item < total;
            const int src = leaf < 0 ? lane : leaf;
            const int g = __shfl(w_geo, src), q = __shfl(w_par, src), cs = __shfl(w_cs, src), first = __shfl(excl, src);
            if (work) {
                const int logB = q & 255, sub = item - first, b = sub & ((1 << logB) - 1), r = sub >> logB;
                const int blen = g >> 16;
                const i32 c = (i32)(i16)(cs & 0xffff), sn = (i32)(i16)(cs >> 16);
                i16 *const p0 = xv + (g & 0xffff) + b * blen;
                const i32 cc = pass == 0 ? sn : c, ss = pass == 0 ? c : sn;
                rotate_chain(p0, r, blen, pass == 0 ? q >> 8 : 1, rot_pack(cc, -ss), rot_pack(ss, cc));
            }
            OG_LSYNC();
        }
    }
}
#endif

#ifdef OG_RECON_TIGHT
constexpr int PVQ_MAIN_LEN = ROM_PVQ_RB9, PVQ_TOP0_OFF = (X_TOP0 - V_NORM) / 2, PVQ_TOP1_OFF = (X_TOP1 - V_NORM) / 2;
static_assert((ROM_PVQ_RB12 - ROM_PVQ_RB9) * 2 <= 160 && (ROM_PVQ_RR_LEN - ROM_PVQ_RB12) * 2 + 32 <= 160, "the short rows (and the rotation marker) fit the tops");
#else
constexpr int PVQ_MAIN_LEN = ROM_PVQ_RR_LEN;
#endif
struct PvqLds {
    u32 rr[PVQ_MAIN_LEN];
    i16 rb[16];
    OG_MEMBER u32 at(int i) const { return reinterpret_cast<const u32 *>(this)[i]; }
};
OG_DEV int pvq_lds_index(int t) {
#ifdef OG_RECON_TIGHT
    return t < ROM_PVQ_RB9 ? t : t < ROM_PVQ_RB12 ? t - ROM_PVQ_RB9 + PVQ_TOP0_OFF : t - ROM_PVQ_RB12 + PVQ_TOP1_OFF;
#else
    return t;
#endif
}
#ifdef OG_RECON_TIGHT
static_assert(sizeof(PvqLds) <= (V_JOBM - V_NORM) * 2, "the PVQ table's long rows end before the jobs' collapse masks");
#else
static_assert(sizeof(PvqLds) <= (V_TOTAL - V_NORM) * 2, "the PVQ table overlays the folding-history, pulse and scratch rows");
#endif
OG_DEV PvqLds &pvq_lds() { return *reinterpret_cast<PvqLds *>(&S.v[V_NORM]); }
OG_DEV void pvq_tab_load() {
    u32 *const dst = reinterpret_cast<u32 *>(&pvq_lds());
#ifdef OG_HOST_EMUL
    OG_FOR_LANES(t, ROM_PVQ_RR_LEN) dst[pvq_lds_index(t)] = rom_pvq_rr[t];
    OG_FOR_LANES(t, 16) pvq_lds().rb[t] = (i16)pvq_lds_index(rom_pvq_rb[t]);
#else
    constexpr int NRR = (ROM_PVQ_RR_LEN + OG_NLANES - 1) / OG_NLANES;
    u32 rr[NRR];
#pragma unroll
    for (int k = 0; k < NRR; k++) rr[k] = rom_pvq_rr[OG_MIN(OG_LANE + k * OG_NLANES, ROM_PVQ_RR_LEN - 1)];
    const u16 rb = rom_pvq_rb[OG_LANE & 15];
#pragma unroll
    for (int k = 0; k < NRR; k++)
        if (OG_LANE + k * OG_NLANES < ROM_PVQ_RR_LEN) dst[pvq_lds_index(OG_LANE + k * OG_NLANES)] = rr[k];
    if (OG_LANE < 16) pvq_lds().rb[OG_LANE] = (i16)pvq_lds_index((int)rb);
#endif
}
OG_DEV u32 pvq_row_sel(int r, u32 v2, u32 v3) {
    u32 v = (u32)(r >= 1);
    v = r == 2 ? v2 : v;
    return r == 3 ? v3 : v;
}
#ifdef OG_HOST_EMUL
OG_DEV u32 pvq_u3(u32 h) { return 2u * h * (h - 1u) + 1u; }
OG_DEV int pvq_isqrt_near(u32 tq) { return (int)__builtin_sqrtf((float)tq); }
#else
OG_DEV u32 pvq_u3(u32 h) {
    u32 r;
    const u32 a = h << 1, b = h - 1u;
    asm("v_mad_u32_u24 %0, %1, %2, 1" : "=v"(r) : "v"(a), "v"(b));
    return r;
}
OG_DEV int pvq_isqrt_near(u32 tq) { return (int)__builtin_amdgcn_sqrtf((float)tq); }
#endif
#ifdef OG_HOST_EMUL
OG_DEV u32 pvq_block_mul(int blen) { return blen > 0 ? 65536u / (u32)blen + 1u : 0u; }
OG_DEV int pvq_block_of(int j, u32 mul) { return (int)(((u32)j * mul) >> 16); }
#else
OG_DEV u32 pvq_block_mul(int blen) { return (u32)(65536.0f * __builtin_amdgcn_rcpf((float)blen)) + 1u; }
OG_DEV int pvq_block_of(int j, u32 mul) { return (int)(__umul24((u32)j, mul) >> 16); }
#endif
OG_DEV int pvq_row_base(const PvqLds &T, int r) { return (int)T.rb[r < 4 ? 4 : (r > 14 ? 14 : r)]; }

OG_DEV u32 pvq_leaf_lane(i16 *xv, const PvqLds &T, int n, int k, u32 i, int pos, int B, i32 gain, int spread, RotJob *defer = nullptr) {
    const int N = n, K = k, x = pos;
    const int logB = ilog2(B), blen = N >> logB;
    i32 yy = 0;
    const u32 bmul = pvq_block_mul(blen);
    u32 cm = 0;
    OG_MARK(56);
    int b0 = pvq_row_base(T, k), b1 = pvq_row_base(T, k + 1);
    while (n > 2) {
        if (k == 0) break;
        u32 h = (u32)n, v2 = 2u * h - 1u, v3 = pvq_u3(h);
        const bool sparse = n > k;
        u32 p0, p1;
        int bn = 0;
        bool tab = false;
        if (sparse) {
            const u32 c0 = T.at(k >= 4 ? b0 + n : 0), c1 = T.at(k >= 3 ? b1 + n : 0);
            p0 = k >= 4 ? c0 : pvq_row_sel(k, v2, v3);
            p1 = k >= 3 ? c1 : pvq_row_sel(k + 1, v2, v3);
            if (k <= 13 && n > k && n > 3) {
                const u32 Vn = p0 + p1, t = Vn - i, m = i >= t ? i - t + 1u : t - i;
                const int lo0 = k + 1 > 2 ? k + 1 : 2;
                int a;
                u32 t0 = p0, t1 = p1;
                if (k <= 2) {
                    const u32 tq = (m + 1u) >> 1;
                    int r = (int)tq;
                    if (k == 2) {
                        r = pvq_isqrt_near(tq);
                        r += (u32)(r * r) < tq;
                    }
                    a = r > lo0 ? r : lo0;
                    const u32 u2 = 2u * (u32)a - 1u;
                    t0 = k == 1 ? 1u : u2;
                    t1 = k == 1 ? u2 : pvq_u3((u32)a);
                } else {
                    int lo = lo0, hi = n;
                    while (lo < hi) {
                        const int mid = (lo + hi) >> 1;
                        const u32 m0 = T.at(k >= 4 ? b0 + mid : 0), m1 = T.at(b1 + mid);
                        const u32 a0 = k >= 4 ? m0 : pvq_u3((u32)mid);
                        if (a0 + m1 >= m) {
                            hi = mid;
                            t0 = a0;
                            t1 = m1;
                        } else
                            lo = mid + 1;
                    }
                    a = lo;
                }
                if (a < n) {
                    i -= (Vn - (t0 + t1)) >> 1;
                    pos += n - a;
                    n = a;
                    if (n <= 2) break;
                    h = (u32)n;
                    v2 = 2u * h - 1u;
                    v3 = pvq_u3(h);
                    p0 = t0;
                    p1 = t1;
                }
            }
        } else {
            const u32 hk = (u32)k;
            bn = pvq_row_base(T, n);
            tab = n >= 4;
            const u32 a0 = T.at(tab ? bn + k : 0), a1 = T.at(tab ? bn + k + 1 : 0);
            p0 = tab ? a0 : pvq_u3(hk);
            p1 = tab ? a1 : pvq_u3(hk + 1u);
        }
        const int s = -(int)(i >= p1);
        i -= p1 & (u32)s;
        if (p0 <= i && s == 0) {
            i -= p0;
        } else {
            u32 plo = 0;
            const bool tabp = sparse || tab;
            const int off = sparse ? n : bn;
            int lo = sparse ? OG_MIN(3, k - 1) : 0, hi = k - 1;
            while (lo < hi) {
                const int mid = (lo + hi + 1) >> 1;
                const int rbm = pvq_row_base(T, mid);
                const u32 tm = T.at(tabp ? (sparse ? rbm : mid) + off : 0);
                const u32 pm = tabp ? tm : pvq_u3((u32)mid);
                if (pm <= i) {
                    lo = mid;
                    plo = pm;
                } else
                    hi = mid - 1;
            }
            int kk = lo;
            if (sparse && lo <= 3) {
                const u32 cand[3] = {1u, v2, v3};
                kk = 0;
#pragma unroll
                for (int r = 1; r <= 3; r++) {
                    const bool ok = r < k && cand[r - 1] <= i;
                    kk = ok ? r : kk;
                    plo = ok ? cand[r - 1] : plo;
                }
            }
            const int val = (k - kk + s) ^ s;
            k = kk;
            i -= plo;
            xv[pos] = (i16)val;
            cm |= 1u << pvq_block_of(pos - x, bmul);
            yy += val * val;
            b0 = pvq_row_base(T, k);
            b1 = pvq_row_base(T, k + 1);
        }
        pos++;
        n--;
    }
    {
        const u32 p = 2 * (u32)k + 1;
        int s = -(int)(i >= p);
        i -= p & (u32)s;
        const int k0 = k;
        k = (int)((i + 1) >> 1);
        if (k) i -= 2 * (u32)k - 1;
        int val = (k0 - k + s) ^ s;
        xv[pos] = (i16)val;
        cm |= (u32)(val != 0) << pvq_block_of(pos - x, bmul);
        pos++;
        yy += val * val;
        s = -(int)i;
        val = (k + s) ^ s;
        xv[pos] = (i16)val;
        cm |= (u32)(val != 0) << pvq_block_of(pos - x, bmul);
        yy += val * val;
    }
#ifdef OG_PVQ_WALK_TAP
    OG_PVQ_WALK_TAP(xv + x, N, yy);
#endif
    OG_MARK(57);
    cm = B > 1 ? cm & ((1u << B) - 1u) : 1u;
    OG_MARK(58);
    const int kk = ilog2(yy) >> 1;
    const i32 t = vshr32(yy, 2 * (kk - 7));
    const i32 g = tr16(mul16_p15(rsqrt_norm(t), gain));
    for (int j = 0; j < N; j++) xv[x + j] = (i16)pshr32(mul16(g, xv[x + j]), kk + 1);
    OG_MARK(59);
    if (2 * K < N && spread != 0) {
        const int factor = spread == 1 ? 15 : (spread == 2 ? 10 : 5);
        const i32 rg = tr16(mul32_q31(mul16(32767, N), celt_rcp(N + factor * K)));
        const i32 theta = tr16(mul16_q15(rg, rg) >> 1);
        const i32 c = cos_norm(theta), s = cos_norm(sub16(32767, theta));
        int stride2 = 0;
        if (N >= 8 * B) {
            stride2 = 1;
            while ((stride2 * stride2 + stride2) * B + (B >> 2) < N) stride2++;
        }
        if (defer) {
            defer->x = x;
            defer->blen = blen;
            defer->logB = logB;
            defer->stride2 = stride2;
            defer->c = c;
            defer->s = s;
            defer->on = true;
            return cm;
        }
        for (int blk2 = 0; blk2 < B; blk2++) {
            if (stride2) rotate1_lane(xv, x + blk2 * blen, blen, stride2, s, c);
            rotate1_lane(xv, x + blk2 * blen, blen, 1, c, s);
        }
    }
    return cm;
}

OG_DEV void job_mask_or(int job, u32 m) {
#ifdef OG_HOST_EMUL
    S.job_mask_row()[job] |= m;
#else
    __hip_atomic_fetch_or(&S.job_mask_row()[job], m, __ATOMIC_RELAXED, __HIP_MEMORY_SCOPE_WORKGROUP);
#endif
}

constexpr int REC_WORDS_CAP = (REC_MAX_WORDS + 64) / 64 * 64;
struct RecCur {
    const u32 *words;
    int w, base, leaf;
};
OG_DEV u32 rec_word(RecCur &cur) {
    if ((unsigned)(cur.w - cur.base) >= 64u) {
        OG_LSYNC();
        OG_FOR_LANES(l, 64) S.word_window()[l] = cur.words[OG_MIN(cur.w + l, REC_WORDS_CAP - 1)];
        OG_LSYNC();
        cur.base = cur.w;
    }
    const u32 w = (u32)OG_UNI(S.word_window()[cur.w - cur.base]);
    cur.w++;
    return w;
}

OG_DEV void rec_word4(RecCur &cur, u32 &w0, u32 &w1, u32 &w2, u32 &w3) {
    const int at = cur.w - cur.base;
    if (at >= 0 && at <= 60) {
        const u32 *win = S.word_window();
        const u32 a = win[at], b = win[at + 1], c = win[at + 2], d = win[at + 3];
        w0 = (u32)OG_UNI(a);
        w1 = (u32)OG_UNI(b);
        w2 = (u32)OG_UNI(c);
        w3 = (u32)OG_UNI(d);
        cur.w += 4;
        return;
    }
    w0 = rec_word(cur);
    w1 = rec_word(cur);
    w2 = rec_word(cur);
    w3 = rec_word(cur);
}

struct LcgTab {
    OG_MEMBER u32 at(u32 seed, int j) const {
        const u32 a = rom_lcg_jump[2 * j], c = rom_lcg_jump[2 * j + 1];
        return a * seed + c;
    }
};

OG_DEV void anti_collapse_pm(const LcgTab &lcg, int LM, int C, int size, int start, int end, u32 seed) {
    i16 *const rrow = &S.v[V_TMP];
    OG_LSYNC();
    OG_FOR_LANES(l, C * NBANDS) {
        const int c = l >= NBANDS ? 1 : 0, i = l - c * NBANDS;
        i32 r = 0;
        if (i >= start && i < end) {
            const int N0 = rom_eband[i + 1] - rom_eband[i];
            const int depth = (int)(udiv((u32)(1 + S.pulses_row()[i]), (u32)N0) >> LM);
            const i32 thresh32 = celt_exp2(-shl16(depth, 10 - BITRES)) >> 1;
            const i32 thresh = tr16(mul16x32_q15(16384, OG_MIN(32767, thresh32)));
            i32 t = N0 << LM;
            const int shift = ilog2(t) >> 1;
            t = shl32(t, (7 - shift) << 1);
            const i32 sqrt_1 = rsqrt_norm(t);
            i32 prev1 = S.logE1_row()[c * NBANDS + i], prev2 = S.logE2_row()[c * NBANDS + i];
            if (C == 1) {
                prev1 = OG_MAX(prev1, (i32)S.logE1_row()[NBANDS + i]);
                prev2 = OG_MAX(prev2, (i32)S.logE2_row()[NBANDS + i]);
            }
            i32 Ediff = (i32)S.bandE_row()[c * NBANDS + i] - OG_MIN(prev1, prev2);
            Ediff = OG_MAX(0, Ediff);
            if (Ediff < 16384) {
                const i32 r32 = celt_exp2(-tr16(Ediff)) >> 1;
                r = tr16(2 * OG_MIN(16383, r32));
            }
            if (LM == 3) r = tr16(mul16_q14(23170, OG_MIN(23169, r)));
            r = tr16(OG_MIN(thresh, r) >> 1);
            r = tr16(mul16_q15(sqrt_1, r) >> shift);
        }
        rrow[l] = (i16)r;
    }
    OG_LSYNC();
    for (int i = start; i < end; i++) {
        const int N0 = rom_eband[i + 1] - rom_eband[i];
        for (int c = 0; c < C; c++) {
            const i32 r = (i32)OG_UNI(rrow[c * NBANDS + i]);
            const int x = V_X + c * size + (rom_eband[i] << LM);
            int renorm = 0;
            const u32 mask = (u32)OG_UNI(S.cmask_row()[i * C + c]);
            for (int k = 0; k < 1 << LM; k++) {
                if (!(mask & (1u << k))) {
                    OG_LSYNC();
                    OG_FOR_LANES(j, N0) S.v[x + (j << LM) + k] = (i16)((lcg.at(seed, j) & 0x8000) ? r : -r);
                    seed = lcg_skip(seed, (u32)N0);
                    renorm = 1;
                }
            }
            if (renorm) renormalise(x, N0 << LM, 32767);
        }
    }
}

OG_DEV u32 recon_job_leaves(RecCur &cur, const LcgTab &lcg, u32 jw, u32 &seed_io, int x_job, int low_job, i32 fill_job, int job) {
    const int n_fill = (int)(jw & 31), n_pvq = (int)(jw >> JW_NPVQ_SHIFT) & 31;
    u32 cm_job = n_pvq ? (u32)OG_UNI(S.job_mask_row()[job]) : 0u;
    for (int f = 0; f < n_fill; f++) {
        OG_MARK(7);
        const u32 w = rec_word(cur), w1 = rec_word(cur);
        const int off = (int)(w >> LW_OFF_SHIFT) & 15, B = ((int)(w >> LW_B_SHIFT) & 15) + 1, N = (int)(w >> LW_N_SHIFT) & 255;
        const int x = V_X + (int)(w1 & 2047);
        const i32 gain = (i32)((w1 >> 11) & 0xffff);
        const u32 cm_mask = (u32)((1ull << B) - 1);
        const i32 fill = (i32)((u32)(fill_job >> off) & cm_mask);
        OG_STAT(10, fill == 0);
        OG_STAT(11, fill != 0 && low_job < 0);
        OG_STAT(12, fill != 0 && low_job >= 0);
        if (fill) {
            const u32 seed = seed_io;
            u32 cm;
            OG_LSYNC();
            if (low_job < 0) {
                OG_FOR_LANES(j, N) S.v[x + j] = (i16)((i32)lcg.at(seed, j) >> 20);
                cm = cm_mask;
            } else {
                const int low = low_job + (x - x_job);
                OG_FOR_LANES(j, N) S.v[x + j] = (i16)(S.v[low + j] + ((lcg.at(seed, j) & 0x8000) ? 4 : -4));
                cm = (u32)fill;
            }
            seed_io = lcg_skip(seed, (u32)N);
            renormalise(x, N, gain);
            cm_job |= cm << off;
        }
        OG_MARK(6);
    }
    return cm_job;
}

OG_DEV void haar1_p2(int x, int N0, int log_stride) {
    N0 >>= 1;
    const int stride = 1 << log_stride;
    OG_LSYNC();
    OG_FOR_LANES(id, N0 << log_stride) {
        const int j = id >> log_stride, i = id & (stride - 1);
        const int a = x + stride * 2 * j + i, b = a + stride;
        const i32 t1 = mul16(23170, S.v[a]), t2 = mul16(23170, S.v[b]);
        S.v[a] = (i16)pshr32(t1 + t2, 15);
        S.v[b] = (i16)pshr32(t1 - t2, 15);
    }
    OG_LSYNC();
}
OG_DEV void hadamard_p2(int x, int N0, int log_stride, int hadamard, int dir) {
    const int stride = 1 << log_stride, N = N0 << log_stride;
    OG_LSYNC();
    OG_FOR_LANES(inter, N) {
        const int j = inter >> log_stride, i = inter & (stride - 1);
        const int blocked = (hadamard ? ordery(stride, i) : i) * N0 + j;
        if (dir == 0)
            S.v[V_TMP + blocked] = S.v[x + inter];
        else
            S.v[V_TMP + inter] = S.v[x + blocked];
    }
    OG_LSYNC();
    OG_FOR_LANES(id, N) S.v[x + id] = S.v[V_TMP + id];
    OG_LSYNC();
}

OG_DEV u32 recon_band_mono(RecCur &cur, u32 jw, const LcgTab &lcg, int tf_change, u32 &seed, int x, int N, int B, int low, int low_out,
                           i32 scale, int low_scratch, i32 fill, int job) {
    const int N0 = N, longBlocks = B == 1;
    int logB = ilog2(B), time_divide = 0, recombine = 0;
    int N_B = N >> logB;
    OG_STAT(1, 1);
    OG_STAT(2, (jw & JW_NEED_LOW) && low >= 0);
    OG_STAT(3, (int)(jw & 31));
    OG_STAT(4, (int)(jw >> JW_NPVQ_SHIFT) & 31);
    OG_STAT(5, tf_change != 0);
    OG_STAT(6, B > 1);
    if (!(jw & JW_NEED_LOW)) low = -1;
    if (tf_change > 0) recombine = tf_change;
    if (low_scratch >= 0 && low >= 0 && (recombine || ((N_B & 1) == 0 && tf_change < 0) || B > 1)) {
        OG_LSYNC();
        OG_FOR_LANES(j, N) S.v[low_scratch + j] = S.v[low + j];
        OG_LSYNC();
        low = low_scratch;
    }
    for (int k = 0; k < recombine; k++) {
        if (low >= 0) haar1_p2(low, N >> k, k);
        int lo = fill & 0xF, hi = fill >> 4;
        int tl = (lo & 3 ? 1 : 0) | (lo & 12 ? 2 : 0), th = (hi & 3 ? 1 : 0) | (hi & 12 ? 2 : 0);
        fill = tl | th << 2;
    }
    logB -= recombine;
    N_B <<= recombine;
    while ((N_B & 1) == 0 && tf_change < 0) {
        if (low >= 0) haar1_p2(low, N_B, logB);
        fill |= fill << (1 << logB);
        logB++;
        N_B >>= 1;
        time_divide++;
        tf_change++;
    }
    const int logB0 = logB, N_B0 = N_B, B0 = 1 << logB0;
    if (B0 > 1 && low >= 0) hadamard_p2(low, N_B >> recombine, logB0 + recombine, longBlocks, 0);
    OG_MARK(6);
    u32 cm = recon_job_leaves(cur, lcg, jw, seed, x, low, fill, job);
    OG_MARK(8);
    if (B0 > 1) hadamard_p2(x, N_B >> recombine, logB0 + recombine, longBlocks, 1);
    OG_STAT(7, B0 > 1);
    OG_STAT(8, time_divide + recombine);
    OG_STAT(9, low_out >= 0);
    N_B = N_B0;
    for (int k = 0; k < time_divide; k++) {
        logB--;
        N_B <<= 1;
        cm |= cm >> (1 << logB);
        haar1_p2(x, N_B, logB);
    }
    for (int k = 0; k < recombine; k++) {
        u32 c4 = cm & 0xF;
        cm = ((c4 & 1) * 0x03) | ((c4 >> 1 & 1) * 0x0C) | ((c4 >> 2 & 1) * 0x30) | ((c4 >> 3 & 1) * 0xC0);
        haar1_p2(x, N0 >> k, k);
    }
    logB += recombine;
    OG_MARK(9);
    if (low_out >= 0) {
        OG_LSYNC();
        OG_FOR_LANES(j, N0) S.v[low_out + j] = (i16)mul16_q15(scale, S.v[x + j]);
        OG_LSYNC();
    }
    return cm & ((1u << (1 << logB)) - 1);
}

OG_DEV void recon_all_bands(const u32 *words, u32 need_norm, const LcgTab &lcg, int start, int end, int C, int N_ch, int shortBlocks, int LM,
                            u32 &seed_io) {
    const int M = 1 << LM, B = shortBlocks ? M : 1;
    OG_STAT(0, 1);
    OG_STAT(19, shortBlocks != 0);
    const int norm_offset = M * rom_eband[start];
    const int norm = V_NORM, norm2 = V_NORM + M * rom_eband[NBANDS - 1] - norm_offset;
    int low_scratch = V_IY;
    RecCur cur;
    cur.words = words;
    cur.w = 0;
    cur.base = -64;
    cur.leaf = 0;
    u32 seed = seed_io;
    for (int i = start; i < end; i++) {
        OG_MARK(3);
        const int last = i == end - 1;
        u32 w0, w1, w2, w3;
        cur.w = (cur.w + 3) & ~3;
        rec_word4(cur, w0, w1, w2, w3);
        const int eb0 = (int)(w1 >> 11) & 2047, N = (int)(w1 >> 22) & 255;
        const int x = V_X + eb0, y = C == 2 ? V_X + N_ch + eb0 : -1;
        const int dual_stereo = (w0 & BW_DUAL) != 0;
        if (i == start + 1) {
            int n1 = M * (rom_eband[start + 1] - rom_eband[start]), n2 = M * (rom_eband[start + 2] - rom_eband[start + 1]);
            if (n2 > n1) {
                OG_LSYNC();
                OG_FOR_LANES(j, n2 - n1) {
                    S.v[norm + n1 + j] = S.v[norm + 2 * n1 - n2 + j];
                    if (w0 & BW_DUAL_PRE) S.v[norm2 + n1 + j] = S.v[norm2 + 2 * n1 - n2 + j];
                }
                OG_LSYNC();
            }
        }
        const int tf_change = (int)((w0 >> BW_TF_SHIFT) & 7) - 4;
        OG_STAT(13, 1);
        OG_STAT(14, N == 1);
        OG_STAT(15, (w0 & BW_STEREO) && N > 2);
        OG_STAT(16, (w0 & BW_STEREO) && N == 2);
        OG_STAT(17, dual_stereo);
        OG_STAT(18, (w0 & BW_HAS_LOW) != 0);
        if (last) low_scratch = -1;
        u32 x_cm, y_cm;
        if (w0 & BW_HAS_LOW) {
            const int fold_end = (int)(w0 >> BW_FOLD1_SHIFT) & 31;
            int fold_i = (int)(w0 >> BW_FOLD0_SHIFT) & 31;
            x_cm = y_cm = 0;
            do {
                x_cm |= (u32)OG_UNI(S.cmask_row()[fold_i * C + 0]);
                y_cm |= (u32)OG_UNI(S.cmask_row()[fold_i * C + C - 1]);
            } while (++fold_i < fold_end);
        } else
            x_cm = y_cm = (1u << B) - 1;
        if (w0 & BW_DUAL_END) {
            OG_LSYNC();
            OG_FOR_LANES(j, eb0 - norm_offset) S.v[norm + j] = (i16)((S.v[norm + j] + S.v[norm2 + j]) >> 1);
            OG_LSYNC();
        }
        const int eff = (w0 & BW_HAS_LOW) ? (int)(w1 & 2047) : -1;
        const int low1 = eff >= 0 ? norm + eff : -1, low2 = eff >= 0 ? norm2 + eff : -1;
        const int want_out = !last && ((need_norm >> i) & 1u);
        const int out1 = want_out ? norm + eb0 - norm_offset : -1, out2 = want_out ? norm2 + eb0 - norm_offset : -1;

        if (N == 1) {
            OG_MARK(11);
            OG_LSYNC();
            S.v[x] = (i16)((w0 & BW_SIGN0) ? -16384 : 16384);
            if (y >= 0) S.v[y] = (i16)((w0 & BW_SIGN1) ? -16384 : 16384);
            OG_LSYNC();
            if (out1 >= 0) S.v[out1] = (i16)(S.v[x] >> 4);
            if (dual_stereo && out2 >= 0) S.v[out2] = (i16)(S.v[y] >> 4);
            OG_LSYNC();
            x_cm = y_cm = 1;
        } else {
            OG_MARK(4);
            const int stereo = (w0 & BW_STEREO) != 0, mid_first = (w0 & BW_MID_FIRST) != 0, swap_c = (w0 & BW_SWAP) != 0;
            const i32 imid = (i32)(i16)(w2 & 0xffff), iside = (i32)(w2 >> 16), scale = (i32)(i16)(w3 & 0xffff);
            i32 fill0 = (i32)(x_cm | y_cm);
            const i32 orig_fill = fill0;
            int n2case = 0, njobs = 1;
            if (stereo) {
                if (w0 & BW_THETA0) fill0 &= (1 << B) - 1;
                if (w0 & BW_THETA1) fill0 &= ((1 << B) - 1) << B;
                if (N == 2)
                    n2case = 1;
                else
                    njobs = 2;
            } else if (dual_stereo)
                njobs = 2;
            u32 cm0 = 0, cm1 = 0;
#pragma nounroll
            for (int jb = 0; jb < njobs; jb++) {
                int jx, jlow, jout, jscr;
                i32 jfill;
                if (dual_stereo) {
                    jx = jb ? y : x; jlow = jb ? low2 : low1; jout = jb ? out2 : out1; jscr = low_scratch;
                    jfill = (i32)(jb ? y_cm : x_cm);
                } else if (!stereo) {
                    jx = x; jlow = low1; jout = out1; jscr = low_scratch; jfill = fill0;
                } else if (n2case) {
                    jx = swap_c ? y : x; jlow = low1; jout = out1; jscr = low_scratch; jfill = orig_fill;
                } else if ((jb == 0) == (mid_first != 0)) {
                    jx = x; jlow = low1; jout = out1; jscr = low_scratch; jfill = fill0;
                } else {
                    jx = y; jlow = -1; jout = -1; jscr = -1; jfill = fill0 >> B;
                }
                OG_MARK(5);
                const u32 jw = rec_word(cur);
                const u32 cmj = recon_band_mono(cur, jw, lcg, tf_change, seed, jx, N, B, jlow, jout, scale, jscr, jfill, 2 * i + jb);
                if (jb == 0) cm0 = cmj; else cm1 = cmj;
            }
            OG_MARK(10);
            if (stereo) {
                if (n2case) {
                    const int x2 = swap_c ? y : x, sign = (w0 & BW_SIGN) ? -1 : 1;
                    OG_LSYNC();
                    const i32 a0 = S.v[x2], a1 = S.v[x2 + 1];
                    const i32 b0 = tr16(-sign * a1), b1 = tr16(sign * a0);
                    i32 X0 = swap_c ? b0 : a0, X1 = swap_c ? b1 : a1, Y0 = swap_c ? a0 : b0, Y1 = swap_c ? a1 : b1;
                    X0 = tr16(mul16_q15(imid, X0));
                    X1 = tr16(mul16_q15(imid, X1));
                    Y0 = tr16(mul16_q15(iside, Y0));
                    Y1 = tr16(mul16_q15(iside, Y1));
                    OG_LSYNC();
                    S.v[x] = (i16)sub16(X0, Y0);
                    S.v[y] = (i16)add16(X0, Y0);
                    S.v[x + 1] = (i16)sub16(X1, Y1);
                    S.v[y + 1] = (i16)add16(X1, Y1);
                    OG_LSYNC();
                } else
                    stereo_merge(x, y, imid, N);
                if (w0 & BW_INV) {
                    OG_LSYNC();
                    OG_FOR_LANES(j, N) S.v[y + j] = (i16)(-S.v[y + j]);
                    OG_LSYNC();
                }
                x_cm = y_cm = cm0 | cm1;
            } else if (dual_stereo) {
                x_cm = cm0;
                y_cm = cm1;
            } else
                x_cm = y_cm = cm0;
        }
        S.cmask_row()[i * C + 0] = (u8)x_cm;
        S.cmask_row()[i * C + C - 1] = (u8)y_cm;
    }
    seed_io = seed;
}

}

#include "og_celt_recon_pm.hpp"

namespace og {

enum { RECON_ALL = 0, RECON_FAST_ONLY = 1, RECON_REST_ONLY = 2, RECON_NOT_MINE = -1000 };

struct ReconHdr {
    i32 ret;
    u32 rng_final, flags;
    i32 pf_pitch, pf_gain, pf_tapset, start, n_leaves, n_words, n_coef;
    u32 need_norm;
    i32 channels, prev_mode, frames_decoded;
    u32 rng;
    i32 ring_pos, st_pf_period, st_pf_period_old, st_pf_gain, st_pf_gain_old, st_pf_tapset, st_pf_tapset_old;
};
OG_DEV void recon_hdr_load(const StreamState *st, const ParseRec *rec, ReconHdr &h) {
    h.ret = OG_UNI(rec->ret); h.rng_final = (u32)OG_UNI(rec->rng_final); h.flags = (u32)OG_UNI(rec->flags);
    h.pf_pitch = OG_UNI(rec->pf_pitch); h.pf_gain = OG_UNI(rec->pf_gain); h.pf_tapset = OG_UNI(rec->pf_tapset);
    h.start = OG_UNI(rec->start); h.n_leaves = OG_UNI(rec->n_leaves); h.n_words = OG_UNI(rec->n_words);
    h.need_norm = (u32)OG_UNI(rec->need_norm); h.n_coef = OG_UNI(rec->n_coef);
    h.channels = OG_UNI(st->channels); h.prev_mode = OG_UNI(st->prev_mode); h.frames_decoded = OG_UNI(st->frames_decoded);
    const CeltState *cs = &st->celt;
    h.rng = (u32)OG_UNI(cs->rng); h.ring_pos = OG_UNI(cs->ring_pos);
    h.st_pf_period = OG_UNI(cs->pf_period); h.st_pf_period_old = OG_UNI(cs->pf_period_old);
    h.st_pf_gain = OG_UNI(cs->pf_gain); h.st_pf_gain_old = OG_UNI(cs->pf_gain_old);
    h.st_pf_tapset = OG_UNI(cs->pf_tapset); h.st_pf_tapset_old = OG_UNI(cs->pf_tapset_old);
}
#ifndef OG_HOST_EMUL
static_assert(offsetof(ParseRec, ret) == 0 && offsetof(ParseRec, rng_final) == 4 && offsetof(ParseRec, flags) == 8 && offsetof(ParseRec, pf_pitch) == 16 &&
              offsetof(ParseRec, pf_gain) == 20 && offsetof(ParseRec, pf_tapset) == 24 && offsetof(ParseRec, start) == 28 &&
              offsetof(ParseRec, n_leaves) == 32 && offsetof(ParseRec, n_words) == 36 && offsetof(ParseRec, need_norm) == 40 &&
              offsetof(ParseRec, n_coef) == 44, "record header words");
static_assert(offsetof(StreamState, channels) == 0 && offsetof(StreamState, prev_mode) == 4, "stream header words");
static_assert(offsetof(CeltState, rng) == offsetof(CeltState, deemph) + 8 && offsetof(CeltState, ring_pos) == offsetof(CeltState, deemph) + 12 &&
              offsetof(CeltState, pf_period) == offsetof(CeltState, deemph) + 16 && offsetof(CeltState, pf_tapset_old) == offsetof(CeltState, deemph) + 36,
              "stream scalar words");
OG_DEV i32 recon_hdr_fetch(const StreamState *st, const ParseRec *rec) {
    const int l = OG_LANE;
    const i32 *p = l < 16 ? reinterpret_cast<const i32 *>(rec) + l
                 : l < 20 ? reinterpret_cast<const i32 *>(st) + (l - 16)
                          : reinterpret_cast<const i32 *>(&st->celt.deemph[0]) + ((l < 32 ? l : 31) - 20);
    return *p;
}
OG_DEV void recon_hdr_unpack(i32 w, ReconHdr &h) {
#define OG_HW(lane) __builtin_amdgcn_readlane(w, lane)
    h.ret = OG_HW(0); h.rng_final = (u32)OG_HW(1); h.flags = (u32)OG_HW(2); h.pf_pitch = OG_HW(4); h.pf_gain = OG_HW(5); h.pf_tapset = OG_HW(6);
    h.start = OG_HW(7); h.n_leaves = OG_HW(8); h.n_words = OG_HW(9); h.need_norm = (u32)OG_HW(10); h.n_coef = OG_HW(11);
    h.channels = OG_HW(16); h.prev_mode = OG_HW(17); h.frames_decoded = OG_HW(18);
    h.rng = (u32)OG_HW(22); h.ring_pos = OG_HW(23); h.st_pf_period = OG_HW(24); h.st_pf_period_old = OG_HW(25); h.st_pf_gain = OG_HW(26);
    h.st_pf_gain_old = OG_HW(27); h.st_pf_tapset = OG_HW(28); h.st_pf_tapset_old = OG_HW(29);
#undef OG_HW
}
#endif

struct ReconCtx {
    ReconHdr h;
    u32 flags, rng_final;
    int ret, mode, C;
    int mode_after = -1;
    bool leaves;
    bool fast;
    bool was_reset = false;
    bool booked = false;
    bool pre = false;
    i32 pre_bandE, pre_logE1, pre_logE2, pre_pulses;
};
OG_DEV bool recon_fast_eligible(const ReconHdr &h) {
    if (h.flags & (RF_SKIP | RF_BAD_CELT)) return false;
    return ((h.flags >> RF_LM_SHIFT) & 3) == 3 && h.n_words < REC_MAX_WORDS && h.n_leaves <= FAST_MAX_LEAVES;
}
OG_DEV bool recon_begin(StreamState *st, const ParseRec *rec, int mode, int ch, int role, ReconCtx &rx) {
    rx.flags = rx.h.flags;
    rx.ret = rx.h.ret;
    rx.mode = mode;
    rx.C = ch;
    rx.leaves = false;
    if (rx.flags & RF_SKIP) {
        if (role == RECON_FAST_ONLY) rx.ret = (int)RECON_NOT_MINE;
        return false;
    }
    rx.fast = recon_fast_eligible(rx.h);
    if ((role == RECON_FAST_ONLY && !rx.fast) || (role == RECON_REST_ONLY && rx.fast)) {
        rx.ret = (int)RECON_NOT_MINE;
        return false;
    }
    const int prev_mode = rx.h.prev_mode;
    if (mode != prev_mode && prev_mode > 0) {
        celt_reset_state(&st->celt);
        rx.was_reset = true;
        rx.h.rng = 0;
        rx.h.st_pf_period = rx.h.st_pf_period_old = rx.h.st_pf_tapset = rx.h.st_pf_tapset_old = 0;
        rx.h.st_pf_gain = rx.h.st_pf_gain_old = 0;
        OG_LSYNC();
    }
    rx.rng_final = rx.h.rng_final;
    if (!(rx.flags & RF_BAD_CELT)) {
        rx.leaves = true;
        OG_MARK(1);
        OG_LSYNC();
#ifndef OG_RECON_TIGHT
        CeltState *cs = &st->celt;
        OG_FOR_LANES(i, 2 * NBANDS) {
            S.bandE_row()[i] = rec->bandE[i];
            S.logE1_row()[i] = cs->logE1[i];
            S.logE2_row()[i] = cs->logE2[i];
            S.cmask_row()[i] = 0;
        }
        OG_FOR_LANES(i, NBANDS) {
            S.pulses_row()[i] = rec->pulses[i];
            S.tf_res[i] = rec->tf_res[i];
        }
#endif
        OG_FOR_LANES(i, 2 * NBANDS) S.job_mask_row()[i] = 0;
#ifdef OG_HOST_EMUL
        OG_FOR_LANES(i, 2 * 960) S.v[V_X + i] = 0;
#else
        OG_FOR_LANES(i, 2 * 960 / 8) *reinterpret_cast<og_v4i *>(&S.v[V_X + 8 * i]) = og_v4i{0, 0, 0, 0};
#endif
    }
    return true;
}

OG_DEV void recon_leaves_own(const ParseRec *rec, const ReconCtx &rx, bool pre = false, u32 g0 = 0, u32 aux0 = 0, u32 idx0 = 0) {
    const int n_leaves = rx.h.n_leaves, spread = (int)(rx.flags >> RF_SPREAD_SHIFT) & 3;
#if defined(OG_HOST_EMUL) && defined(OG_STATS)
    {
        int max_n = 0, k_at_max = 0, sum_n = 0;
        for (int t = 0; t < n_leaves; t++) {
            const u32 g = rec->leaf[t].geom;
            const int n = (int)(g >> 11) & 255, k = (int)(g >> 19) & 255;
            sum_n += n;
            if (n > max_n) { max_n = n; k_at_max = k; }
        }
        OG_STAT(40, max_n); OG_STAT(41, k_at_max); OG_STAT(42, sum_n); OG_STAT(44, n_leaves);
        OG_STAT(45, max_n >= 96); OG_STAT(46, max_n >= 144);
    }
#endif
    OG_MARK(2);
#ifdef OG_HOST_EMUL
    OG_FOR_LANES(t, n_leaves) {
        const bool first = pre && t < OG_NLANES;
        const u32 g = first ? g0 : rec->leaf[t].geom;
        const u32 aux = first ? aux0 : rec->leaf[t].aux;
        const u32 idx = first ? idx0 : rec->leaf[t].idx;
        job_mask_or((int)(aux >> 20) & 63, (pvq_leaf_lane(S.v, pvq_lds(), (int)(g >> 11) & 255, (int)(g >> 19) & 255, idx, V_X + (int)(g & 2047),
                                                          (int)(g >> 27) + 1, (i32)(aux & 0xffff), spread)
                                            << ((aux >> 16) & 15)) & 0xffffu);
    }
    OG_LSYNC();
#else
    for (int t0 = 0; t0 < n_leaves; t0 += OG_NLANES) {
        const int t = t0 + OG_LANE;
        RotJob job;
        job.x = job.blen = job.logB = job.stride2 = 0;
        job.c = job.s = 0;
        job.on = false;
        if (t < n_leaves) {
            const bool first = pre && t0 == 0;
            const u32 g = first ? g0 : rec->leaf[t].geom;
            const u32 aux = first ? aux0 : rec->leaf[t].aux;
            const u32 idx = first ? idx0 : rec->leaf[t].idx;
            job_mask_or((int)(aux >> 20) & 63, (pvq_leaf_lane(S.v, pvq_lds(), (int)(g >> 11) & 255, (int)(g >> 19) & 255, idx, V_X + (int)(g & 2047),
                                                              (int)(g >> 27) + 1, (i32)(aux & 0xffff), spread, &job)
                                                << ((aux >> 16) & 15)) & 0xffffu);
        }
        OG_LSYNC();
        OG_MARK(28);
        pvq_rotate_wave(S.v, job, S.rot_marker());
    }
    OG_LSYNC();
#endif
}

OG_DEV int recon_result(const ReconCtx &rx) { return (rx.leaves && (rx.flags & RF_TELL_OVERFLOW)) ? INTERNAL_ERROR : rx.ret; }
OG_DEV void recon_bookkeeping(StreamState *st, const ReconCtx &rx) {
    if (OG_LANE == 0) {
        st->prev_mode = rx.mode_after >= 0 ? rx.mode_after : rx.mode;
        st->frames_decoded = rx.h.frames_decoded + 1;
        st->range_final = rx.rng_final;
    }
}
OG_DEV int recon_finish(StreamState *st, const ParseRec *rec, const ReconCtx &rx) {
    const u32 flags = rx.flags;
    const int mode = rx.mode, C = rx.C, CC = rx.h.channels;
    int result = rx.ret;
    if (rx.leaves) {
        const int LM = (int)(flags >> RF_LM_SHIFT) & 3, M = 1 << LM, N = M * 120;
        const int transient = (flags & RF_TRANSIENT) != 0, silence = (flags & RF_SILENCE) != 0;
        const int start = rx.h.start, end = NBANDS;
        CeltState *cs = &st->celt;
        LcgTab lcg;
#ifndef OG_RECON_TIGHT
        const bool pm = rx.fast;
        if (!pm) {
            OG_FOR_LANES(i, 1248) S.v[V_NORM + i] = 0;
            OG_LSYNC();
        }
#endif
        u32 seed = rx.h.rng;
#ifdef OG_RECON_TIGHT
        recon_all_bands_pm(rec, lcg, C, transient ? M : 0, seed, start);
        if (rx.pre) {
            if (OG_LANE < 2 * NBANDS) {
                S.bandE_row()[OG_LANE] = (i16)rx.pre_bandE;
                S.logE1_row()[OG_LANE] = (i16)(rx.was_reset ? -28 * 1024 : rx.pre_logE1);
                S.logE2_row()[OG_LANE] = (i16)(rx.was_reset ? -28 * 1024 : rx.pre_logE2);
            }
            if (OG_LANE < NBANDS) S.pulses_row()[OG_LANE] = rx.pre_pulses;
        } else {
            OG_FOR_LANES(i, 2 * NBANDS) {
                S.bandE_row()[i] = rec->bandE[i];
                S.logE1_row()[i] = cs->logE1[i];
                S.logE2_row()[i] = cs->logE2[i];
            }
            OG_FOR_LANES(i, NBANDS) S.pulses_row()[i] = rec->pulses[i];
        }
        OG_LSYNC();
#else
        if (pm)
            recon_all_bands_pm(rec, lcg, C, transient ? M : 0, seed, start);
        else
            recon_all_bands(rec->words, rx.h.need_norm, lcg, start, end, C, N, transient ? M : 0, LM, seed);
#endif
        OG_MARK(12);
        if (flags & RF_ANTI_COLLAPSE) anti_collapse_pm(lcg, LM, C, N, start, end, seed);
        if (silence) {
            OG_LSYNC();
            OG_FOR_LANES(i, C * NBANDS) S.bandE_row()[i] = (i16)(-28 * 1024);
        }
        OG_TAP(1);
        CeltSynth sp;
        sp.N = N; sp.LM = LM; sp.C = C; sp.CC = CC; sp.start = start; sp.end = end; sp.silence = silence; sp.transient = transient;
        sp.pf_pitch = rx.h.pf_pitch; sp.pf_tapset = rx.h.pf_tapset; sp.pf_gain = rx.h.pf_gain;
        sp.have_state = 1;
        sp.st_pf_period = rx.h.st_pf_period; sp.st_pf_period_old = rx.h.st_pf_period_old; sp.st_pf_gain = rx.h.st_pf_gain;
        sp.st_pf_gain_old = rx.h.st_pf_gain_old; sp.st_pf_tapset = rx.h.st_pf_tapset; sp.st_pf_tapset_old = rx.h.st_pf_tapset_old;
        sp.st_ring_pos = rx.h.ring_pos;
        sp.rng_final = rx.rng_final; sp.rc_error = (flags & RF_RC_ERROR) != 0; sp.inline_deemph = 0;
        sp.loss = nullptr; sp.lost = 0; sp.energies_kept_by_parse = 1;
        OG_MARK(13);
        celt_synthesis(cs, sp);
        OG_MARK(17);
        if (flags & RF_TELL_OVERFLOW) result = INTERNAL_ERROR;
    }
    if (!rx.booked) recon_bookkeeping(st, rx);
    return result;
}

OG_DEV int celt_recon_wave(StreamState *st, const ParseRec *rec, int mode, int ch, int role = RECON_ALL, int mode_after = -1) {
    ReconCtx rx;
    rx.mode_after = mode_after;
    recon_hdr_load(st, rec, rx.h);
    if (!recon_begin(st, rec, mode, ch, role, rx)) return rx.ret;
    if (rx.leaves) {
        pvq_tab_load();
        OG_LSYNC();
        recon_leaves_own(rec, rx);
    }
    return recon_finish(st, rec, rx);
}

OG_DEV void celt_post(StreamState *st, const ParseRec *rec, int result, int c, i16 *pcm, const i16 *silk, int ch) {
    if (rec->flags & (RF_SKIP | RF_BAD_CELT)) return;
    celt_post_lane(&st->celt, c, st->channels, 960, (st->celt.ring_pos - 960) & RING_MASK, result >= 0 ? pcm : nullptr, silk, 960 * ch);
}

}
```

### esp32-opus-player_amd/csrc/og_ctx.hpp

```cpp
#pragma once
#include <hip/hip_runtime_api.h>
#include <stdint.h>
#include <stdio.h>
#include <condition_variable>
#include <functional>
#include <mutex>
#include <thread>
#include <utility>
#include <vector>
#include "../../include/opusgpu.h"
#include "og_debug.hpp"

namespace og {
struct StreamState;
}
enum { OPUSGPU_COPY_PIECES = 16, OPUSGPU_COPY_THREADS = 8 };

struct HostPool {
    std::vector<std::thread> th;
    std::mutex m;
    std::condition_variable wake, done;
    std::function<void(int)> job;
    int generation = 0, want = 0, pending = 0;
    bool quit = false;
    ~HostPool() {
        {
            std::lock_guard<std::mutex> l(m);
            quit = true;
        }
        wake.notify_all();
        for (auto &t : th) t.join();
    }
    void worker(int id) {
        int seen = 0;
        for (;;) {
            std::function<void(int)> f;
            {
                std::unique_lock<std::mutex> l(m);
                wake.wait(l, [&] { return quit || (generation != seen && id < want); });
                if (quit) return;
                seen = generation;
                f = job;
            }
            f(id);
            {
                std::lock_guard<std::mutex> l(m);
                if (--pending == 0) done.notify_all();
            }
        }
    }
    void run(int count, const std::function<void(int)> &f) {
        if (count <= 1) {
            f(0);
            return;
        }
        while ((int)th.size() < count - 1) {
            const int id = (int)th.size();
            th.emplace_back([this, id] { worker(id); });
        }
        {
            std::lock_guard<std::mutex> l(m);
            job = [&f](int id) { f(id + 1); };
            want = count - 1;
            pending = count - 1;
            generation++;
        }
        wake.notify_all();
        f(0);
        std::unique_lock<std::mutex> l(m);
        done.wait(l, [&] { return pending == 0; });
    }
};

struct opusgpu_ctx {
    int device = -1;
    hipStream_t stream = nullptr;
    og::StreamState *d_streams = nullptr;
    int n_streams = 0, channels = 0;
    void *d_descs = nullptr, *d_arena = nullptr, *d_pcm = nullptr, *d_result = nullptr;
    size_t cap_descs = 0, cap_arena = 0, cap_pcm = 0, cap_result = 0;
    void *h_pcm = nullptr, *h_res = nullptr;
    size_t cap_h_pcm = 0, cap_h_res = 0;
    void *h_arena = nullptr, *h_descs = nullptr;
    size_t cap_h_arena = 0, cap_h_descs = 0;
    HostPool pool;
    uint32_t *d_crc_tables = nullptr;
    hipEvent_t ev_piece[OPUSGPU_COPY_PIECES] = {};
    hipStream_t copy_stream = nullptr;
    std::mutex registered_mutex;
    std::vector<std::pair<uintptr_t, size_t>> registered;
    hipEvent_t ev_part[OPUSGPU_COPY_PIECES] = {};
    int host_parts = 8;
    void *d_recs[6] = {}, *d_rout[6] = {};
    size_t cap_recs[6] = {}, cap_rout[6] = {};
    void *d_handoff[OG_SILK_SETS] = {}, *d_srecs[OG_SILK_SETS] = {};
    size_t cap_handoff[OG_SILK_SETS] = {}, cap_srecs[OG_SILK_SETS] = {};
    const void *last_srecs = nullptr;
    void *d_shadow = nullptr;
    StepPipeline sp;
    int split_celt = 1;
    int split_hybrid = 1;
    int fast_recon = 1;
    int mode = OPUSGPU_MODE_REFERENCE;
    int pipeline = 0;
    long long stall_ticks = 0;
    const void *last_recs = nullptr;
    int parse_groups = 1;
    const void *last_descs = nullptr;
    int last_n = 0, last_had_silk_recs = 0;
    std::vector<int32_t> last_count, last_flags;
    char err[256] = {0};
};

static int fail(opusgpu_ctx *ctx, int code, const char *what, hipError_t e) {
    if (ctx) snprintf(ctx->err, sizeof(ctx->err), "%s: %s", what, hipGetErrorString(e));
    return code;
}
#define HIPCHK(ctx, call)                                                \
    do {                                                                 \
        hipError_t e_ = (call);                                          \
        if (e_ != hipSuccess) return fail(ctx, OPUSGPU_ERR_HIP, #call, e_); \
    } while (0)
static int grow(opusgpu_ctx *ctx, void **p, size_t *cap, size_t need);
```

### esp32-opus-player_amd/csrc/og_debug.hpp

```cpp
#pragma once
#include <stdlib.h>
#include <string.h>

struct og_debug_knobs {
    int split = 1, split_hybrid = 1, fast_recon = 1, hybrid_recon_aside = 1, silk_params_aside = 1, silk_nb_kernel = 1, halves = 1, silk_pipeline = 1, hybrid_pipeline = 1, parse_wide = 1, parse_groups = 1, parse_priority = 1, host_parts = 16, host_slices = 1, host_timing = 0,
        pages_timing = 0, launch_delay_us = 0, stall_stream = 0, stall_us = 0;
};
inline const og_debug_knobs &og_debug() {
    static const og_debug_knobs k = [] {
        og_debug_knobs v;
        auto flag = [](const char *name, int &field) {
            if (const char *e = getenv(name)) field = e[0] != '0' && e[0] != '\0';
        };
        auto number = [](const char *name, int &field, int lo, int hi) {
            if (const char *e = getenv(name)) {
                const int x = atoi(e);
                if (x >= lo && x <= hi) field = x;
            }
        };
        flag("OPUSGPU_SPLIT", v.split);
        flag("OPUSGPU_SPLIT_HYBRID", v.split_hybrid);
        flag("OPUSGPU_FAST_RECON", v.fast_recon);
        number("OPUSGPU_HYBRID_RECON_ASIDE", v.hybrid_recon_aside, 0, 2);
        flag("OPUSGPU_SILK_PARAMS_ASIDE", v.silk_params_aside);
        flag("OPUSGPU_SILK_NB_KERNEL", v.silk_nb_kernel);
        flag("OPUSGPU_HALVES", v.halves);
        flag("OPUSGPU_SILK_PIPELINE", v.silk_pipeline);
        flag("OPUSGPU_HYBRID_PIPELINE", v.hybrid_pipeline);
        number("OPUSGPU_PARSE_WIDE", v.parse_wide, 0, 2);
        number("OPUSGPU_PARSE_GROUPS", v.parse_groups, 1, 8);
        flag("OPUSGPU_PARSE_PRIORITY", v.parse_priority);
        if (const char *e = getenv("OPUSGPU_HOST_PARTS")) {
            const int x = atoi(e);
            if (x == 1 || x == 2 || x == 4 || x == 8 || x == 16) v.host_parts = x;
        }
        flag("OPUSGPU_HOST_SLICES", v.host_slices);
        if (const char *e = getenv("OPUSGPU_HOST_TIMING")) v.host_timing = atoi(e) == 2 ? 2 : 1;
        v.pages_timing = getenv("OPUSGPU_PAGES_TIMING") != nullptr;
        number("OPUSGPU_LAUNCH_DELAY_US", v.launch_delay_us, 0, 100000);
        if (const char *e = getenv("OPUSGPU_STALL_STREAM")) {
            const char *names[] = {"step", "parse", "recon", "side"};
            for (int i = 0; i < 4; i++)
                if (!strcmp(e, names[i])) v.stall_stream = i + 1;
        }
        if (const char *e = getenv("OPUSGPU_STALL_US")) {
            const int x = atoi(e);
            v.stall_us = x < 0 ? 0 : x > 100000 ? 100000 : x;
        }
        if (!v.stall_stream || !v.stall_us) v.stall_stream = v.stall_us = 0;
        return v;
    }();
    return k;
}
```

### esp32-opus-player_amd/csrc/og_recon.hip

```cpp
#define OG_RECON_TIGHT 1
#include <hip/hip_runtime.h>
#include "og_celt_recon.hpp"

using namespace og;

#define OG_FAST_WAVES 6


__global__ void __launch_bounds__(64, OG_FAST_WAVES) k_celt_recon_fb(const FrameDesc *__restrict__ descs, StreamState *st,
                                                                           const ParseRec *recs, ReconOut *rout, int n, int n_streams,
                                                                           int hybrid, u32 *started) {
    if (started && threadIdx.x == 0 && (blockIdx.x & 63) == 0) __hip_atomic_fetch_add(started, 1u, __ATOMIC_RELAXED, __HIP_MEMORY_SCOPE_SYSTEM);
    const int f = (int)blockIdx.x;
    StreamState *sp = nullptr;
    const ParseRec *rec = nullptr;
    ReconCtx rx;
    rx.leaves = false;
    rx.flags = 0;
    bool mine = false;
    int pos = 0;
    u32 lg = 0, la = 0, li = 0;
    OG_PROF_INIT();
    if (f < n) {
        rec = &recs[f];
        const FrameDesc d = descs[f];
        const int lane = OG_LANE;
        const i32 w_rec = reinterpret_cast<const i32 *>(rec)[lane < 16 ? lane : 15];
        {
            typedef u32 u32x4 __attribute__((ext_vector_type(4)));
            const u32x4 lf = *reinterpret_cast<const u32x4 *>(&rec->leaf[lane]);
            li = lf[0];
            lg = lf[1];
            la = lf[2];
        }
        rx.pre_bandE = rec->bandE[lane < 2 * NBANDS ? lane : 0];
        rx.pre_pulses = rec->pulses[lane < NBANDS ? lane : 0];
        const int mode = desc_mode(d.flags);
        bool ok = !(d.stream < 0 || d.stream >= n_streams || !(mode == MODE_CELT || (mode == MODE_HYBRID && hybrid)) || desc_rfc(d.flags));
        if (ok) {
            sp = &st[d.stream];
            const i32 w_st = recon_hdr_fetch(sp, rec);
            rx.pre_logE1 = sp->celt.logE1[lane < 2 * NBANDS ? lane : 0];
            rx.pre_logE2 = sp->celt.logE2[lane < 2 * NBANDS ? lane : 0];
            rx.pre = true;
            recon_hdr_unpack(lane < 16 ? w_rec : w_st, rx.h);
            if (mode == MODE_HYBRID && (rx.h.flags & RF_SKIP)) ok = false;
        }
        if (ok) {
            pos = rx.h.ring_pos;
            mine = recon_begin(sp, rec, mode, desc_channels(d.flags), RECON_FAST_ONLY, rx);
            if (mine) {
                if (OG_LANE == 0) rout[f] = ReconOut{recon_result(rx), pos};
                recon_bookkeeping(sp, rx);
                rx.booked = true;
            }
        }
    }
    if (mine && rx.leaves) {
        pvq_tab_load();
        OG_SYNC();
        recon_leaves_own(rec, rx, true, lg, la, li);
    }
    if (mine) recon_finish(sp, rec, rx);
    OG_PROF_FLUSH();
}

extern "C" void og_launch_celt_recon_fb(hipStream_t s, const void *descs, void *streams, const void *recs, void *rout, int n,
                                        int n_streams, int hybrid, unsigned *started) {
    hipLaunchKernelGGL(k_celt_recon_fb, dim3(n), dim3(64), 0, s, (const FrameDesc *)descs, (StreamState *)streams,
                       (const ParseRec *)recs, (ReconOut *)rout, n, n_streams, hybrid, started);
}
extern "C" int og_celt_recon_fb_signals(int n) { return (n + 63) / 64; }

#ifdef OG_PROF
extern "C" int og_recon_fb_prof(unsigned long long *out64, int reset) {
    if (hipMemcpyFromSymbol(out64, HIP_SYMBOL(g_prof), sizeof(unsigned long long) * 64) != hipSuccess) return -1;
    if (reset) {
        unsigned long long z[64] = {0};
        if (hipMemcpyToSymbol(HIP_SYMBOL(g_prof), z, sizeof(z)) != hipSuccess) return -1;
    }
    return 0;
}
#endif
```

### esp32-opus-player_amd/csrc/og_step.hpp

```cpp
#pragma once
#include <hip/hip_runtime_api.h>
#include <stddef.h>
#include <stdint.h>
#include <algorithm>
#include <chrono>
#include <functional>
#include <thread>

#define OG_SILK_SETS 3
static_assert(OG_SILK_SETS >= 2, "a pipelined SILK / hybrid step runs next to the step before it");

struct StepPipeline {
    int slot = 0, front_recorded = 0, post_recorded[3] = {};
    hipStream_t parse_stream = nullptr, recon_stream = nullptr, last_step_stream = nullptr;
    hipStream_t side_stream = nullptr;
    hipEvent_t ev_fork = nullptr, ev_join = nullptr;
    hipEvent_t ev_front = nullptr;
    hipEvent_t ev_parsed = nullptr;
    hipEvent_t ev_recon = nullptr;
    hipEvent_t ev_post[3] = {};
    unsigned shadow_epoch = 1;
    int silk_slot = 0, sdone_recorded[OG_SILK_SETS] = {}, last_silk_mask = 0, last_kind = 0;
    bool last_kind2_celt = false;
    hipEvent_t ev_sparsed = nullptr, ev_sdone[OG_SILK_SETS] = {}, ev_sp = nullptr, ev_spar = nullptr, ev_hrecon = nullptr;
    uint32_t *d_started = nullptr;
    uint32_t parse_started_total = 0, recon_started_total = 0;
    uint32_t window_parse_target = 0, window_recon_target = 0;

    void drained() {
        front_recorded = post_recorded[0] = post_recorded[1] = post_recorded[2] = 0;
        for (int i = 0; i < OG_SILK_SETS; i++) sdone_recorded[i] = 0;
        last_silk_mask = 0;
    }
};

#include "og_ctx.hpp"

struct Step {
    hipStream_t s;
    int n;
    const void *descs, *arena;
    void *pcm, *result;
    int pcm_stride, modes;
    bool keeps_kind, any_silk, any_celt;
    int sset;
    void *recs, *rout, *handoff, *srecs;
};

void launch_stream_stall(opusgpu_ctx *ctx, hipStream_t q);
void launch_decode_rfc(opusgpu_ctx *ctx, hipStream_t q, const Step &st);
void launch_decode_step(opusgpu_ctx *ctx, hipStream_t q, const Step &st, size_t f0, int cnt, int pass);
void launch_silk_parse(opusgpu_ctx *ctx, hipStream_t q, const Step &st, size_t f0, int cnt, void *shadow, uint32_t epoch);
void launch_silk_parse64(opusgpu_ctx *ctx, hipStream_t q, const Step &st, size_t f0, int cnt, void *shadow, uint32_t epoch);
void launch_silk_params(opusgpu_ctx *ctx, hipStream_t q, const Step &st, size_t f0, int cnt, void *shadow, uint32_t epoch);
void launch_celt_parse(opusgpu_ctx *ctx, hipStream_t q, const Step &st, size_t f0, int cnt, bool wide, bool early);
int celt_parse_early_grid(const opusgpu_ctx *ctx, int cnt, bool wide);
void launch_celt_recon_fb(opusgpu_ctx *ctx, hipStream_t q, const Step &st, size_t f0, int cnt, bool counts_in);
extern "C" int og_celt_recon_fb_signals(int n);
void launch_celt_recon(opusgpu_ctx *ctx, hipStream_t q, const Step &st, size_t f0, int cnt);
void launch_celt_post(opusgpu_ctx *ctx, hipStream_t q, const Step &st, size_t f0, int cnt, bool others);
void launch_silk_synth(opusgpu_ctx *ctx, hipStream_t q, const Step &st, size_t f0, int cnt, int nb_done);
void launch_silk_synth_nb(opusgpu_ctx *ctx, hipStream_t q, const Step &st, size_t f0, int cnt);
extern const size_t og_parse_rec_bytes, og_recon_out_bytes, og_silk_handoff_bytes, og_silk_rec_bytes;

static int sync_in_flight(opusgpu_ctx *ctx) {
    if (ctx->sp.parse_stream) {
        HIPCHK(ctx, hipStreamSynchronize(ctx->sp.parse_stream));
        HIPCHK(ctx, hipStreamSynchronize(ctx->sp.recon_stream));
    }
    if (ctx->sp.last_step_stream && ctx->sp.last_step_stream != ctx->stream) HIPCHK(ctx, hipStreamSynchronize(ctx->sp.last_step_stream));
    return OPUSGPU_OK;
}
static int pipeline_create(opusgpu_ctx *ctx) {
    StepPipeline &sp = ctx->sp;
    if (sp.parse_stream) return OPUSGPU_OK;
    int least = 0, greatest = 0;
    HIPCHK(ctx, hipDeviceGetStreamPriorityRange(&least, &greatest));
    if (!og_debug().parse_priority) greatest = least;
    HIPCHK(ctx, hipStreamCreateWithPriority(&sp.parse_stream, hipStreamNonBlocking, greatest));
    HIPCHK(ctx, hipStreamCreateWithFlags(&sp.recon_stream, hipStreamNonBlocking));
    HIPCHK(ctx, hipEventCreateWithFlags(&sp.ev_front, hipEventDisableTiming));
    HIPCHK(ctx, hipEventCreateWithFlags(&sp.ev_parsed, hipEventDisableTiming));
    HIPCHK(ctx, hipEventCreateWithFlags(&sp.ev_recon, hipEventDisableTiming));
    for (int i = 0; i < 3; i++) HIPCHK(ctx, hipEventCreateWithFlags(&sp.ev_post[i], hipEventDisableTiming));
    HIPCHK(ctx, hipMalloc((void **)&sp.d_started, 128));
    HIPCHK(ctx, hipMemset(sp.d_started, 0, 128));
    return OPUSGPU_OK;
}
static void pipeline_destroy(opusgpu_ctx *ctx) {
    StepPipeline &sp = ctx->sp;
    for (hipStream_t q : {sp.parse_stream, sp.recon_stream, sp.side_stream})
        if (q) (void)hipStreamSynchronize(q);
    for (hipEvent_t e : {sp.ev_front, sp.ev_parsed, sp.ev_recon, sp.ev_post[0], sp.ev_post[1], sp.ev_post[2], sp.ev_sparsed, sp.ev_sp, sp.ev_spar,
                         sp.ev_hrecon, sp.ev_fork, sp.ev_join})
        if (e) (void)hipEventDestroy(e);
    for (hipEvent_t e : sp.ev_sdone)
        if (e) (void)hipEventDestroy(e);
    (void)hipFree(sp.d_started);
    for (hipStream_t q : {sp.parse_stream, sp.recon_stream, sp.side_stream})
        if (q) (void)hipStreamDestroy(q);
    sp = StepPipeline();
}
#define OG_SILK_PARSE_WIDE_MIN 98304
#define OG_HALVES_MIN 4096
static void launch_jitter() {
    if (const int us = og_debug().launch_delay_us) std::this_thread::sleep_for(std::chrono::microseconds(us));
}
static int enter_step_kind(opusgpu_ctx *ctx, int kind, hipStream_t s, bool keeps_kind = false, bool celt_frames = false) {
    const bool shares_celt = (kind == 1 && ctx->sp.last_kind == 2 && ctx->sp.last_kind2_celt) || (kind == 2 && celt_frames && ctx->sp.last_kind == 1);
    const bool disjoint = keeps_kind && kind != 0 && ctx->sp.last_kind != 0 && !shares_celt;
    if ((kind == 2) != (ctx->sp.last_kind == 2) && !disjoint) {
        if (int rc = sync_in_flight(ctx)) return rc;
        HIPCHK(ctx, hipStreamSynchronize(s));
        HIPCHK(ctx, hipStreamSynchronize(ctx->stream));
        ctx->sp.drained();
    }
    if (kind != 2 && !(keeps_kind && kind == 1)) ctx->sp.shadow_epoch++;
    ctx->sp.last_kind = kind;
    if (kind == 2) ctx->sp.last_kind2_celt = celt_frames;
    return OPUSGPU_OK;
}

static int grow_step_slot(opusgpu_ctx *ctx, int par, size_t need) {
    int rc;
    if (ctx->cap_recs[par] < og_parse_rec_bytes * need && (rc = grow(ctx, &ctx->d_recs[par], &ctx->cap_recs[par], og_parse_rec_bytes * need)))
        return rc;
    if (ctx->cap_rout[par] < og_recon_out_bytes * need && (rc = grow(ctx, &ctx->d_rout[par], &ctx->cap_rout[par], og_recon_out_bytes * need)))
        return rc;
    return OPUSGPU_OK;
}

static int grow_silk_set(opusgpu_ctx *ctx, int sset, size_t need, hipStream_t drain) {
    int rc;
    if (ctx->cap_handoff[sset] >= og_silk_handoff_bytes * need && ctx->cap_srecs[sset] >= og_silk_rec_bytes * need) return OPUSGPU_OK;
    if (drain) {
        if ((rc = sync_in_flight(ctx))) return rc;
        HIPCHK(ctx, hipStreamSynchronize(drain));
    }
    if (ctx->cap_handoff[sset] < og_silk_handoff_bytes * need &&
        (rc = grow(ctx, &ctx->d_handoff[sset], &ctx->cap_handoff[sset], og_silk_handoff_bytes * need)))
        return rc;
    if (ctx->cap_srecs[sset] < og_silk_rec_bytes * need && (rc = grow(ctx, &ctx->d_srecs[sset], &ctx->cap_srecs[sset], og_silk_rec_bytes * need)))
        return rc;
    return OPUSGPU_OK;
}

static void release_window_waits(opusgpu_ctx *ctx) {
    if (!ctx->sp.d_started || (!ctx->sp.window_parse_target && !ctx->sp.window_recon_target)) return;
    hipStream_t q = nullptr;
    if (hipStreamCreateWithFlags(&q, hipStreamNonBlocking) == hipSuccess) {
        if (ctx->sp.window_parse_target) (void)hipStreamWriteValue32(q, ctx->sp.d_started, ctx->sp.window_parse_target, 0);
        if (ctx->sp.window_recon_target) (void)hipStreamWriteValue32(q, ctx->sp.d_started + 16, ctx->sp.window_recon_target, 0);
        (void)hipStreamSynchronize(q);
        (void)hipStreamDestroy(q);
    }
    (void)sync_in_flight(ctx);
    (void)hipStreamSynchronize(ctx->stream);
    (void)hipMemset(ctx->sp.d_started, 0, 128);
    ctx->sp.parse_started_total = ctx->sp.recon_started_total = 0;
    ctx->sp.window_parse_target = ctx->sp.window_recon_target = 0;
    (void)hipGetLastError();
}

struct StepSlices {
    int count = 0;
    const size_t *bounds = nullptr;
    std::function<int(int)> after_slice;
};
static void stall(opusgpu_ctx *ctx, const Step &st, hipStream_t q) {
    if (!ctx->stall_ticks) return;
    const int w = og_debug().stall_stream;
    hipStream_t const t = w == 1 ? st.s : w == 2 ? ctx->sp.parse_stream : w == 3 ? ctx->sp.recon_stream : ctx->sp.side_stream;
    if (t && q == t) launch_stream_stall(ctx, q);
}
static void front(opusgpu_ctx *ctx, const Step &st, hipStream_t q, size_t f0, int cnt, void *shadow = nullptr, uint32_t epoch = 0,
                  hipStream_t pq = nullptr) {
    if (st.srecs) {
        stall(ctx, st, q);
        if (shadow || cnt >= OG_SILK_PARSE_WIDE_MIN || og_debug().parse_wide == 2)
            launch_silk_parse64(ctx, q, st, f0, cnt, shadow, epoch);
        else
            launch_silk_parse(ctx, q, st, f0, cnt, shadow, epoch);
        if (pq && pq != q) {
            (void)hipEventRecord(ctx->sp.ev_sp, q);
            (void)hipStreamWaitEvent(pq, ctx->sp.ev_sp, 0);
        }
        stall(ctx, st, pq ? pq : q);
        launch_silk_params(ctx, pq ? pq : q, st, f0, cnt, shadow, epoch);
        if (pq && pq != q) (void)hipEventRecord(ctx->sp.ev_spar, pq);
    }
    if (st.any_celt) stall(ctx, st, q);
    if (st.any_celt && ((shadow && og_debug().parse_wide) || og_debug().parse_wide == 2)) {
        launch_celt_parse(ctx, q, st, f0, cnt, true, false);
    } else if (st.any_celt)
        launch_celt_parse(ctx, q, st, f0, cnt, false, false);
}
static void back_half(opusgpu_ctx *ctx, const Step &st, hipStream_t q, size_t f0, int cnt, hipStream_t rq = nullptr) {
    const int modes = st.modes;
    bool others = false;
    if (st.srecs) {
        const int nb = (modes & 1) && og_debug().silk_nb_kernel;
        stall(ctx, st, q);
        if (nb) launch_silk_synth_nb(ctx, q, st, f0, cnt);
        if (nb) stall(ctx, st, q);
        launch_silk_synth(ctx, q, st, f0, cnt, nb);
        others = true;
    } else if (st.any_silk) {
        stall(ctx, st, q);
        launch_decode_step(ctx, q, st, f0, cnt, 1);
        others = true;
    }
    if (st.any_celt) {
        hipStream_t const r = rq ? rq : q;
        if (rq) {
            (void)hipStreamWaitEvent(rq, ctx->sp.ev_sparsed, 0);
            const int two_back = (st.sset + OG_SILK_SETS - 2) % OG_SILK_SETS;
            if (ctx->sp.sdone_recorded[two_back]) (void)hipStreamWaitEvent(rq, ctx->sp.ev_sdone[two_back], 0);
        }
        stall(ctx, st, r);
        if (ctx->fast_recon) launch_celt_recon_fb(ctx, r, st, f0, cnt, false);
        if (ctx->fast_recon) stall(ctx, st, r);
        launch_celt_recon(ctx, r, st, f0, cnt);
        if (rq) {
            (void)hipEventRecord(ctx->sp.ev_hrecon, rq);
            (void)hipStreamWaitEvent(q, ctx->sp.ev_hrecon, 0);
        }
    }
    if (st.any_celt || !others || modes != 7) {
        stall(ctx, st, q);
        launch_celt_post(ctx, q, st, f0, cnt, others);
    }
    if (st.srecs && (modes & 1)) {
        stall(ctx, st, q);
        launch_decode_step(ctx, q, st, f0, cnt, 2);
    }
}
static int step_single_kernel(opusgpu_ctx *ctx, const Step &st, const StepSlices *slices) {
    if (int rc = enter_step_kind(ctx, 0, st.s)) return rc;
    stall(ctx, st, st.s);
    if (ctx->mode == OPUSGPU_MODE_RFC)
        launch_decode_rfc(ctx, st.s, st);
    else
        launch_decode_step(ctx, st.s, st, 0, st.n, 0);
    HIPCHK(ctx, hipGetLastError());
    if (ctx->mode == OPUSGPU_MODE_RFC && ctx->pipeline) {
        HIPCHK(ctx, hipEventRecord(ctx->sp.ev_front, st.s));
        ctx->sp.front_recorded = 1;
    }
    ctx->sp.last_step_stream = st.s;
    if (ctx->mode != OPUSGPU_MODE_RFC && slices)
        for (int i = 0; i < slices->count; i++)
            if (int rc = slices->after_slice(i)) return rc;
    return OPUSGPU_OK;
}
static int step_pipelined_silk(opusgpu_ctx *ctx, const Step &st) {
    hipStream_t const s = st.s;
    const int n = st.n, modes = st.modes;
    const int sset = st.sset;
    const bool keeps_kind = st.keeps_kind;
    if (!ctx->sp.ev_sparsed) {
        HIPCHK(ctx, hipEventCreateWithFlags(&ctx->sp.ev_sparsed, hipEventDisableTiming));
        HIPCHK(ctx, hipEventCreateWithFlags(&ctx->sp.ev_sp, hipEventDisableTiming));
        HIPCHK(ctx, hipEventCreateWithFlags(&ctx->sp.ev_spar, hipEventDisableTiming));
        HIPCHK(ctx, hipEventCreateWithFlags(&ctx->sp.ev_hrecon, hipEventDisableTiming));
        for (int i = 0; i < OG_SILK_SETS; i++) HIPCHK(ctx, hipEventCreateWithFlags(&ctx->sp.ev_sdone[i], hipEventDisableTiming));
    }
    if (ctx->sp.sdone_recorded[sset]) HIPCHK(ctx, hipStreamWaitEvent(ctx->sp.parse_stream, ctx->sp.ev_sdone[sset], 0));
    const int prev_set = (sset + OG_SILK_SETS - 1) % OG_SILK_SETS;
    if (!keeps_kind && (modes & 2) && (ctx->sp.last_silk_mask & 1) && ctx->sp.sdone_recorded[prev_set])
        HIPCHK(ctx, hipStreamWaitEvent(ctx->sp.parse_stream, ctx->sp.ev_sdone[prev_set], 0));
    ctx->sp.last_silk_mask = modes;
    front(ctx, st, ctx->sp.parse_stream, 0, n, ctx->d_shadow, (uint32_t)ctx->sp.shadow_epoch, og_debug().silk_params_aside ? ctx->sp.recon_stream : nullptr);
    HIPCHK(ctx, hipEventRecord(ctx->sp.ev_sparsed, ctx->sp.parse_stream));
    HIPCHK(ctx, hipStreamWaitEvent(s, ctx->sp.ev_sparsed, 0));
    if (og_debug().silk_params_aside) HIPCHK(ctx, hipStreamWaitEvent(s, ctx->sp.ev_spar, 0));
    back_half(ctx, st, s, 0, n, (og_debug().hybrid_recon_aside == 2 || (og_debug().hybrid_recon_aside && (modes & 6) == 2)) ? ctx->sp.recon_stream : nullptr);
    HIPCHK(ctx, hipEventRecord(ctx->sp.ev_sdone[sset], s));
    ctx->sp.sdone_recorded[sset] = 1;
    HIPCHK(ctx, hipGetLastError());
    return OPUSGPU_OK;
}
static int step_in_order(opusgpu_ctx *ctx, const Step &st, const StepSlices *slices) {
    hipStream_t const s = st.s;
    const int n = st.n;
    if (!slices && n >= 2 * OG_HALVES_MIN && og_debug().halves) {
        if (!ctx->sp.ev_fork) {
            HIPCHK(ctx, hipEventCreateWithFlags(&ctx->sp.ev_fork, hipEventDisableTiming));
            HIPCHK(ctx, hipEventCreateWithFlags(&ctx->sp.ev_join, hipEventDisableTiming));
        }
        if (!ctx->sp.recon_stream && !ctx->sp.side_stream) HIPCHK(ctx, hipStreamCreateWithFlags(&ctx->sp.side_stream, hipStreamNonBlocking));
        hipStream_t const side = ctx->sp.recon_stream ? ctx->sp.recon_stream : ctx->sp.side_stream;
        HIPCHK(ctx, hipEventRecord(ctx->sp.ev_fork, s));
        HIPCHK(ctx, hipStreamWaitEvent(side, ctx->sp.ev_fork, 0));
        const int h = (n / 2 + 63) / 64 * 64;
        front(ctx, st, s, 0, h);
        back_half(ctx, st, s, 0, h);
        front(ctx, st, side, (size_t)h, n - h);
        back_half(ctx, st, side, (size_t)h, n - h);
        HIPCHK(ctx, hipEventRecord(ctx->sp.ev_join, side));
        HIPCHK(ctx, hipStreamWaitEvent(s, ctx->sp.ev_join, 0));
    } else if (slices && slices->count > 1) {
        front(ctx, st, s, 0, n);
        for (int i = 0; i < slices->count; i++) {
            const size_t lo = slices->bounds[i], hi = slices->bounds[i + 1];
            if (hi > lo) back_half(ctx, st, s, lo, (int)(hi - lo));
            if (int rc = slices->after_slice(i)) return rc;
        }
    } else {
        front(ctx, st, s, 0, n);
        back_half(ctx, st, s, 0, n);
    }
    HIPCHK(ctx, hipGetLastError());
    if (ctx->pipeline) {
        HIPCHK(ctx, hipEventRecord(ctx->sp.ev_front, s));
        ctx->sp.front_recorded = 1;
    }
    return OPUSGPU_OK;
}
static int step_pipelined_celt(opusgpu_ctx *ctx, const Step &st, int par, int next_n) {
    hipStream_t const s = st.s;
    const int n = st.n;
    const int par2 = (par + 1) % 3;
    const bool window = next_n > 0;
    if (ctx->sp.front_recorded) HIPCHK(ctx, hipStreamWaitEvent(ctx->sp.parse_stream, ctx->sp.ev_front, 0));
    if (ctx->sp.post_recorded[par]) HIPCHK(ctx, hipStreamWaitEvent(ctx->sp.parse_stream, ctx->sp.ev_post[par], 0));
    const bool wide = og_debug().parse_wide != 0;
    {
        const int grid = celt_parse_early_grid(ctx, n, wide);
        launch_jitter();
        stall(ctx, st, ctx->sp.parse_stream);
        launch_celt_parse(ctx, ctx->sp.parse_stream, st, 0, n, wide, true);
        ctx->sp.parse_started_total += (uint32_t)grid;
    }
    HIPCHK(ctx, hipEventRecord(ctx->sp.ev_parsed, ctx->sp.parse_stream));
    hipStream_t const back = ctx->sp.recon_stream;
    HIPCHK(ctx, hipStreamWaitEvent(back, ctx->sp.ev_parsed, 0));
    if (ctx->sp.post_recorded[par2]) HIPCHK(ctx, hipStreamWaitEvent(back, ctx->sp.ev_post[par2], 0));
    if (window) {
        const int next_grid = celt_parse_early_grid(ctx, next_n, wide);
        ctx->sp.window_parse_target = ctx->sp.parse_started_total + (uint32_t)next_grid;
        HIPCHK(ctx, hipStreamWaitValue32(back, ctx->sp.d_started, ctx->sp.window_parse_target, hipStreamWaitValueGte, 0xffffffffu));
    }
    if (ctx->fast_recon) {
        launch_jitter();
        stall(ctx, st, back);
        launch_celt_recon_fb(ctx, back, st, 0, n, true);
        ctx->sp.recon_started_total += (uint32_t)og_celt_recon_fb_signals(n);
    }
    stall(ctx, st, back);
    launch_celt_recon(ctx, back, st, 0, n);
    HIPCHK(ctx, hipEventRecord(ctx->sp.ev_recon, back));
    HIPCHK(ctx, hipStreamWaitEvent(s, ctx->sp.ev_recon, 0));
    if (window && ctx->fast_recon) {
        const int first_round = std::min(og_celt_recon_fb_signals(next_n), 32);
        ctx->sp.window_recon_target = ctx->sp.recon_started_total + (uint32_t)first_round;
        HIPCHK(ctx, hipStreamWaitValue32(s, ctx->sp.d_started + 16, ctx->sp.window_recon_target, hipStreamWaitValueGte, 0xffffffffu));
    }
    launch_jitter();
    stall(ctx, st, s);
    launch_celt_post(ctx, s, st, 0, n, false);
    HIPCHK(ctx, hipEventRecord(ctx->sp.ev_post[par], s));
    ctx->sp.post_recorded[par] = 1;
    HIPCHK(ctx, hipGetLastError());
    return OPUSGPU_OK;
}

static int decode_step_impl(opusgpu_ctx *ctx, int n, const void *d_descs, const void *d_arena, void *d_pcm, void *d_result,
                            void *hip_stream, bool tables_resident, int modes = 7, int next_n = 0, const StepSlices *slices = nullptr) {
    if (!ctx || n < 0 || !ctx->d_streams) return OPUSGPU_BAD_ARG;
    if (n == 0) return OPUSGPU_OK;
    if (!d_descs || !d_arena || !d_pcm || !d_result) return OPUSGPU_BAD_ARG;
    if ((uintptr_t)d_arena & 15) return OPUSGPU_BAD_ARG;
    StepPipeline &sp = ctx->sp;
    Step st = {};
    st.s = hip_stream ? (hipStream_t)hip_stream : ctx->stream;
    st.n = n, st.descs = d_descs, st.arena = d_arena, st.pcm = d_pcm, st.result = d_result;
    st.pcm_stride = (ctx->mode == OPUSGPU_MODE_RFC ? OPUSGPU_RFC_FRAME_SAMPLES : OPUSGPU_FRAME_SAMPLES) * ctx->channels;
    ctx->last_descs = d_descs;
    ctx->last_n = ctx->mode == OPUSGPU_MODE_RFC || !ctx->split_celt ? 0 : n;
    ctx->last_had_silk_recs = ctx->split_celt && ctx->split_hybrid;
    HIPCHK(ctx, hipSetDevice(ctx->device));
    if (ctx->mode == OPUSGPU_MODE_RFC || !ctx->split_celt) return step_single_kernel(ctx, st, slices);
    st.keeps_kind = (modes & OPUSGPU_STEP_KEEPS_MODE) != 0;
    modes &= 7;
    if (!modes) modes = 7;
    st.modes = modes;
    st.any_silk = (modes & 3) != 0, st.any_celt = (modes & 6) != 0;
    const bool pipe = ctx->pipeline && tables_resident && modes == 4;
    const bool pipe_silk = ctx->pipeline && tables_resident && ((modes & 4) == 0 || st.keeps_kind) && (modes & 3) != 0 && ctx->split_hybrid && !slices &&
                           (modes == 1 ? og_debug().silk_pipeline : og_debug().hybrid_pipeline);
    if (int rc = enter_step_kind(ctx, pipe ? 1 : pipe_silk ? 2 : 0, st.s, st.keeps_kind, (modes & 4) != 0)) return rc;
    if (ctx->pipeline && sp.last_step_stream && sp.last_step_stream != st.s) {
        HIPCHK(ctx, hipStreamSynchronize(sp.last_step_stream));
        if (int rc = sync_in_flight(ctx)) return rc;
        sp.drained();
    }
    sp.last_step_stream = st.s;
    if (pipe) sp.slot = (sp.slot + 1) % 3;
    if (pipe_silk) sp.silk_slot = (sp.silk_slot + 1) % OG_SILK_SETS;
    st.sset = pipe_silk ? sp.silk_slot : 0;
    const int par = pipe ? sp.slot : pipe_silk ? 3 + st.sset : 0;
    if (int rc = grow_step_slot(ctx, par, (size_t)n)) return rc;
    if (ctx->split_hybrid && st.any_silk)
        if (int rc = grow_silk_set(ctx, st.sset, (size_t)n, pipe_silk ? st.s : nullptr)) return rc;
    st.recs = ctx->d_recs[par], st.rout = ctx->d_rout[par];
    st.handoff = ctx->split_hybrid && st.any_silk ? ctx->d_handoff[st.sset] : nullptr;
    st.srecs = ctx->split_hybrid && st.any_silk ? ctx->d_srecs[st.sset] : nullptr;
    ctx->last_recs = st.recs;
    ctx->last_srecs = st.srecs;
    ctx->last_had_silk_recs = st.srecs != nullptr;
    if (pipe_silk) return step_pipelined_silk(ctx, st);
    if (pipe) return step_pipelined_celt(ctx, st, par, next_n);
    return step_in_order(ctx, st, slices);
}

static int decode_window(opusgpu_ctx *ctx, int n_steps, const int32_t *n, int max_n, const void *const *d_descs, const void *const *d_arena,
                         void *const *d_pcm, void *const *d_result, void *hip_stream, int m) {
    if (ctx->sp.d_started && (ctx->sp.parse_started_total > 0x70000000u || ctx->sp.recon_started_total > 0x70000000u)) {
        HIPCHK(ctx, hipSetDevice(ctx->device));
        if (int rc = sync_in_flight(ctx)) return rc;
        HIPCHK(ctx, hipStreamSynchronize(ctx->stream));
        HIPCHK(ctx, hipMemset(ctx->sp.d_started, 0, 128));
        ctx->sp.parse_started_total = ctx->sp.recon_started_total = 0;
    }
    if (ctx->pipeline && m == 4 && ctx->split_celt && ctx->mode != OPUSGPU_MODE_RFC) {
        HIPCHK(ctx, hipSetDevice(ctx->device));
        for (int par = 0; par < 3; par++)
            if (int rc = grow_step_slot(ctx, par, (size_t)max_n)) return rc;
    }
    for (int k = 0; k < n_steps; k++) {
        const int next_n = k + 1 < n_steps ? n[k + 1] : 0;
        const int rc = decode_step_impl(ctx, n[k], d_descs[k], d_arena[k], d_pcm[k], d_result[k], hip_stream, true, m, next_n > 0 ? next_n : 0);
        if (rc) {
            release_window_waits(ctx);
            return rc;
        }
    }
    ctx->sp.window_parse_target = ctx->sp.window_recon_target = 0;
    return OPUSGPU_OK;
}
```

Before: 44.18 million frames/s.

## Split CELT PVQ leaf decoding into a separate size-sorted batched kernel

Adds a new k_celt_pvq kernel that runs on the parse stream. Within each block of 64 frames it gathers all PVQ leaves, bins them by (N,K) with an LDS histogram and prefix sum, and decodes them one leaf per lane into an LDS staging area. The goal is to cut the divergence of the per-frame, wave-level leaf walk in the fast recon kernel. Results go into a per-frame 4 KB LeafOut buffer, and the frame is flagged RF_LEAVES_DONE. The recon kernel then only copies the spectrum and job masks and applies the rotations. The cost is an extra kernel launch, additional global-memory traffic for the leaf outputs, and LDS staging with many workgroup barriers.

```diff
diff --git a/__graft_entry__.py b/__graft_entry__.py
--- a/__graft_entry__.py
+++ b/__graft_entry__.py
@@ -25,7 +25,7 @@
     hipcc = os.environ.get("HIPCC", "/opt/rocm/bin/hipcc")
     out = os.path.join(PKG_DIR, "libopusgpu.so")
     cmd = [hipcc, "--offload-arch=gfx950", "-O3", "-std=c++17", "-fPIC", "-shared",
-           os.path.join(CSRC, "og_api.hip"), os.path.join(CSRC, "og_recon.hip"), os.path.join(CSRC, "og_parse64.hip"), os.path.join(CSRC, "og_rfc.hip"), os.path.join(CSRC, "og_silk_nb.hip"), os.path.join(CSRC, "og_silk_synth.hip"), os.path.join(CSRC, "og_compat.cpp"),
+           os.path.join(CSRC, "og_api.hip"), os.path.join(CSRC, "og_recon.hip"), os.path.join(CSRC, "og_pvq.hip"), os.path.join(CSRC, "og_parse64.hip"), os.path.join(CSRC, "og_rfc.hip"), os.path.join(CSRC, "og_silk_nb.hip"), os.path.join(CSRC, "og_silk_synth.hip"), os.path.join(CSRC, "og_compat.cpp"),
            os.path.join(CSRC, "og_pages.cpp"), os.path.join(CSRC, "og_files.cpp"),
            "-I", os.path.join(ROOT, "include"), "-pthread",
            "-o", out]
diff --git a/esp32-opus-player_amd/csrc/og_api.hip b/esp32-opus-player_amd/csrc/og_api.hip
--- a/esp32-opus-player_amd/csrc/og_api.hip
+++ b/esp32-opus-player_amd/csrc/og_api.hip
@@ -324,7 +324,8 @@
 extern "C" int og_celt_parse64_frames(void);
 
 extern "C" void og_launch_celt_recon_fb(hipStream_t s, const void *descs, void *streams, const void *recs, void *rout, int n,
-                                        int n_streams, int hybrid, unsigned *started);
+                                        int n_streams, int hybrid, unsigned *started, const void *leaf_out);
+extern "C" void og_launch_celt_pvq(hipStream_t s, const void *descs, void *recs, void *leaf_out, int n, int n_streams);
 extern "C" int og_celt_recon_fb_signals(int n);
 extern "C" void og_launch_decode_rfc(hipStream_t s, const void *descs, const void *arena, void *streams, void *pcm, void *result, int n,
                                      int n_streams, int pcm_stride);
@@ -569,7 +570,12 @@
 }
 void launch_celt_recon_fb(opusgpu_ctx *ctx, hipStream_t q, const Step &st, size_t f0, int cnt, bool counts_in) {
     const StepRange r(st, f0);
-    og_launch_celt_recon_fb(q, r.dd, ctx->d_streams, r.recs, r.rout, cnt, ctx->n_streams, r.hh ? 1 : 0, counts_in ? ctx->sp.d_started + 16 : nullptr);
+    og_launch_celt_recon_fb(q, r.dd, ctx->d_streams, r.recs, r.rout, cnt, ctx->n_streams, r.hh ? 1 : 0, counts_in ? ctx->sp.d_started + 16 : nullptr,
+                            st.leaf_out ? (const char *)st.leaf_out + f0 * og_leaf_out_bytes : nullptr);
+}
+void launch_celt_pvq(opusgpu_ctx *ctx, hipStream_t q, const Step &st, size_t f0, int cnt) {
+    const StepRange r(st, f0);
+    og_launch_celt_pvq(q, r.dd, r.recs, (char *)st.leaf_out + f0 * og_leaf_out_bytes, cnt, ctx->n_streams);
 }
 void launch_celt_recon(opusgpu_ctx *ctx, hipStream_t q, const Step &st, size_t f0, int cnt) {
     const StepRange r(st, f0);
@@ -614,6 +620,7 @@
     ctx->split_celt = og_debug().split;
     ctx->split_hybrid = og_debug().split_hybrid;
     ctx->fast_recon = og_debug().fast_recon;
+    ctx->pvq_kernel = og_debug().pvq_kernel;
     ctx->parse_groups = og_debug().parse_groups;
     ctx->host_parts = og_debug().host_parts;
     if (og_debug().stall_us) {
@@ -647,6 +654,7 @@
         (void)hipFree(ctx->d_recs[i]);
         (void)hipFree(ctx->d_rout[i]);
     }
+    for (void *p : ctx->d_leaf_out) (void)hipFree(p);
     for (int i = 0; i < OG_SILK_SETS; i++) {
         (void)hipFree(ctx->d_handoff[i]);
         (void)hipFree(ctx->d_srecs[i]);
diff --git a/esp32-opus-player_amd/csrc/og_celt_pvq.hpp b/esp32-opus-player_amd/csrc/og_celt_pvq.hpp
--- /dev/null
+++ b/esp32-opus-player_amd/csrc/og_celt_pvq.hpp
@@ -0,0 +1,130 @@
+#pragma once
+#include "og_celt_recon.hpp"
+
+namespace og {
+
+constexpr int PVQ_BLOCK = 64;
+constexpr int PVQ_REF_CAP = 3840;
+constexpr int PVQ_BINS = 1024;
+constexpr int PVQ_STAGE = 2048;
+static_assert(FAST_MAX_LEAVES < 512 && PVQ_BLOCK <= 64, "a leaf reference is frame << 9 | leaf in 16 bits");
+static_assert(PVQ_STAGE >= 255 && PVQ_STAGE % 8 == 0, "the largest N a leaf word can name fits a lane's staging column");
+
+OG_DEV int pvq_sort_key(int n, int k) {
+    const int cn = n <= 16 ? n : OG_MIN(16 + ((n - 16) >> 3), 31), ck = k <= 23 ? k : OG_MIN(24 + ((k - 24) >> 3), 31);
+    return cn * 32 + ck;
+}
+
+struct SpecStage {
+    i16 *row;
+    int mul, off;
+    OG_MEMBER i16 &at(int p) const { return row[p * mul + off]; }
+};
+
+struct PvqBlockLds {
+    PvqLds T;
+    u16 ref[PVQ_REF_CAP];
+    union {
+        alignas(16) u32 hist[PVQ_BINS];
+        alignas(16) i16 stage[PVQ_STAGE];
+    };
+};
+
+#ifndef OG_HOST_EMUL
+OG_DEV void pvq_block_wave(PvqBlockLds &L, const FrameDesc *descs, ParseRec *recs, LeafOut *lout, int n, int n_streams) {
+    typedef u32 u32x4 __attribute__((ext_vector_type(4)));
+    const int lane = OG_LANE, f = lane;
+    {
+        u32 *const dst = reinterpret_cast<u32 *>(&L.T);
+        for (int t = lane; t < ROM_PVQ_RR_LEN; t += OG_NLANES) dst[t] = rom_pvq_rr[t];
+        if (lane < 16) L.T.rb[lane] = (i16)rom_pvq_rb[lane];
+    }
+    for (int i = lane; i < PVQ_BINS; i += OG_NLANES) L.hist[i] = 0;
+    bool take = false;
+    u32 flags = 0;
+    int cnt = 0;
+    if (f < n) {
+        const FrameDesc d = descs[f];
+        if (d.stream >= 0 && d.stream < n_streams && desc_mode(d.flags) == MODE_CELT && !desc_rfc(d.flags)) {
+            ReconHdr h;
+            h.flags = flags = recs[f].flags;
+            h.n_words = recs[f].n_words;
+            h.n_leaves = cnt = recs[f].n_leaves;
+            take = recon_fast_eligible(h) && cnt >= 0;
+        }
+    }
+    if (!take) cnt = 0;
+    if (wave_scan_add(cnt) > PVQ_REF_CAP) take = false, cnt = 0;
+    const int total = wave_sum(cnt);
+    const unsigned long long taken = __ballot(take);
+    OG_LSYNC();
+    for (int pass = 0; pass < 2; pass++) {
+        for (int fr = 0; fr < PVQ_BLOCK; fr++) {
+            if (!((taken >> fr) & 1ull)) continue;
+            if (pass == 0) {
+                u32x4 *const dst = reinterpret_cast<u32x4 *>(&lout[fr]);
+#pragma unroll
+                for (int r = 0; r < (int)sizeof(LeafOut) / 16 / OG_NLANES; r++) dst[lane + r * OG_NLANES] = u32x4{0, 0, 0, 0};
+            }
+            const int nl = __builtin_amdgcn_readlane(cnt, fr);
+            for (int t = lane; t < nl; t += OG_NLANES) {
+                const u32 g = recs[fr].leaf[t].geom;
+                const int key = pvq_sort_key((int)(g >> 11) & 255, (int)(g >> 19) & 255);
+                const u32 at = __hip_atomic_fetch_add(&L.hist[key], 1u, __ATOMIC_RELAXED, __HIP_MEMORY_SCOPE_WORKGROUP);
+                if (pass == 1 && at < (u32)PVQ_REF_CAP) L.ref[at] = (u16)(fr << 9 | t);
+            }
+        }
+        OG_LSYNC();
+        if (pass == 0) {
+            int carry = 0;
+            for (int r = 0; r < PVQ_BINS / OG_NLANES; r++) {
+                const int v = (int)L.hist[r * OG_NLANES + lane], incl = wave_scan_add(v);
+                L.hist[r * OG_NLANES + lane] = (u32)(carry + incl - v);
+                carry += __builtin_amdgcn_readlane(incl, 63);
+            }
+            OG_LSYNC();
+        }
+    }
+    __threadfence();
+    for (int c0 = 0; c0 < total; c0 += OG_NLANES) {
+        const int idx = c0 + lane;
+        bool have = idx < total;
+        const int r = have ? (int)L.ref[idx] : 0, fr = r >> 9, t = r & 511;
+        u32 li = 0, lg = 0, la = 0;
+        if (have) {
+            const u32x4 lf = *reinterpret_cast<const u32x4 *>(&recs[fr].leaf[t]);
+            li = lf[0], lg = lf[1], la = lf[2];
+        }
+        const int x = (int)(lg & 2047), N = (int)(lg >> 11) & 255, K = (int)(lg >> 19) & 255, B = (int)(lg >> 27) + 1;
+        have = have && N >= 2 && x + N <= 2 * 960 && ((la >> 20) & 63) < 2 * NBANDS;
+        const int nmax = __builtin_amdgcn_readlane(wave_scan_max(have ? N : 0), 63);
+        if (nmax == 0) continue;
+        const int per = OG_MIN(OG_NLANES, PVQ_STAGE / nmax);
+        for (int s0 = 0; s0 < OG_NLANES; s0 += per) {
+            OG_LSYNC();
+            for (int i = lane; i < (nmax * per + 7) / 8; i += OG_NLANES) reinterpret_cast<u32x4 *>(L.stage)[i] = u32x4{0, 0, 0, 0};
+            OG_LSYNC();
+            const int col = lane - s0;
+            if (have && col >= 0 && col < per) {
+                const SpecStage xs{L.stage, per, col - x * per};
+                const u32 cm = pvq_leaf_walk(xs, L.T, N, K, li, x, B, (i32)(la & 0xffff));
+                i16 *const out = lout[fr].x + x;
+                if (((x | N) & 7) == 0) {
+                    for (int j = 0; j < N; j += 8) {
+                        u32x4 v;
+#pragma unroll
+                        for (int q = 0; q < 4; q++) v[q] = (u32)(u16)xs.at(x + j + 2 * q) | (u32)(u16)xs.at(x + j + 2 * q + 1) << 16;
+                        *reinterpret_cast<u32x4 *>(out + j) = v;
+                    }
+                } else
+                    for (int j = 0; j < N; j++) out[j] = xs.at(x + j);
+                const u32 m = (cm << ((la >> 16) & 15)) & 0xffffu;
+                if (m) __hip_atomic_fetch_or(&lout[fr].job_mask[(la >> 20) & 63], m, __ATOMIC_RELAXED, __HIP_MEMORY_SCOPE_AGENT);
+            }
+        }
+    }
+    if (take) recs[f].flags = flags | RF_LEAVES_DONE;
+}
+#endif
+
+}
diff --git a/esp32-opus-player_amd/csrc/og_celt_rec.hpp b/esp32-opus-player_amd/csrc/og_celt_rec.hpp
--- a/esp32-opus-player_amd/csrc/og_celt_rec.hpp
+++ b/esp32-opus-player_amd/csrc/og_celt_rec.hpp
@@ -12,7 +12,8 @@
     RF_SILENCE = 1, RF_TRANSIENT = 2, RF_LM_SHIFT = 2 , RF_STEREO = 16, RF_SPREAD_SHIFT = 5 ,
     RF_DUAL = 128, RF_ANTI_COLLAPSE = 256, RF_RC_ERROR = 512, RF_TELL_OVERFLOW = 1024,
     RF_SKIP = 2048,
-    RF_BAD_CELT = 4096
+    RF_BAD_CELT = 4096,
+    RF_LEAVES_DONE = 8192
 };
 enum {
     BW_SIGN0 = 1, BW_SIGN1 = 2, BW_INV = 4, BW_SIGN = 8, BW_MID_FIRST = 16, BW_SWAP = 32,
@@ -66,6 +67,13 @@
 
 constexpr int FAST_MAX_LEAVES = 416;
 
+struct LeafOut {
+    alignas(128) i16 x[2 * 960];
+    u32 job_mask[2 * NBANDS];
+    u32 pad[(4096 - 2 * 2 * 960) / 4 - 2 * NBANDS];
+};
+static_assert(sizeof(LeafOut) == 4096, "a leaf-output slot is 256 pieces of 16 bytes");
+
 struct ReconOut {
     i32 ret, pos;
 };
diff --git a/esp32-opus-player_amd/csrc/og_celt_recon.hpp b/esp32-opus-player_amd/csrc/og_celt_recon.hpp
--- a/esp32-opus-player_amd/csrc/og_celt_recon.hpp
+++ b/esp32-opus-player_amd/csrc/og_celt_recon.hpp
@@ -192,8 +192,13 @@
 #endif
 OG_DEV int pvq_row_base(const PvqLds &T, int r) { return (int)T.rb[r < 4 ? 4 : (r > 14 ? 14 : r)]; }
 
-OG_DEV u32 pvq_leaf_lane(i16 *xv, const PvqLds &T, int n, int k, u32 i, int pos, int B, i32 gain, int spread, RotJob *defer = nullptr) {
-    const int N = n, K = k, x = pos;
+struct SpecArena {
+    i16 *xv;
+    OG_MEMBER i16 &at(int p) const { return xv[p]; }
+};
+template <class Spec>
+OG_DEV u32 pvq_leaf_walk(const Spec xs, const PvqLds &T, int n, int k, u32 i, int pos, int B, i32 gain) {
+    const int N = n, x = pos;
     const int logB = ilog2(B), blen = N >> logB;
     i32 yy = 0;
     const u32 bmul = pvq_block_mul(blen);
@@ -296,7 +301,7 @@
             const int val = (k - kk + s) ^ s;
             k = kk;
             i -= plo;
-            xv[pos] = (i16)val;
+            xs.at(pos) = (i16)val;
             cm |= 1u << pvq_block_of(pos - x, bmul);
             yy += val * val;
             b0 = pvq_row_base(T, k);
@@ -313,18 +318,18 @@
         k = (int)((i + 1) >> 1);
         if (k) i -= 2 * (u32)k - 1;
         int val = (k0 - k + s) ^ s;
-        xv[pos] = (i16)val;
+        xs.at(pos) = (i16)val;
         cm |= (u32)(val != 0) << pvq_block_of(pos - x, bmul);
         pos++;
         yy += val * val;
         s = -(int)i;
         val = (k + s) ^ s;
-        xv[pos] = (i16)val;
+        xs.at(pos) = (i16)val;
         cm |= (u32)(val != 0) << pvq_block_of(pos - x, bmul);
         yy += val * val;
     }
 #ifdef OG_PVQ_WALK_TAP
-    OG_PVQ_WALK_TAP(xv + x, N, yy);
+    OG_PVQ_WALK_TAP(&xs.at(x), N, yy);
 #endif
     OG_MARK(57);
     cm = B > 1 ? cm & ((1u << B) - 1u) : 1u;
@@ -332,9 +337,12 @@
     const int kk = ilog2(yy) >> 1;
     const i32 t = vshr32(yy, 2 * (kk - 7));
     const i32 g = tr16(mul16_p15(rsqrt_norm(t), gain));
-    for (int j = 0; j < N; j++) xv[x + j] = (i16)pshr32(mul16(g, xv[x + j]), kk + 1);
-    OG_MARK(59);
+    for (int j = 0; j < N; j++) xs.at(x + j) = (i16)pshr32(mul16(g, xs.at(x + j)), kk + 1);
+    return cm;
+}
+OG_DEV bool pvq_leaf_rotation(int N, int K, int B, int x, int spread, RotJob &job) {
     if (2 * K < N && spread != 0) {
+        const int logB = ilog2(B), blen = N >> logB;
         const int factor = spread == 1 ? 15 : (spread == 2 ? 10 : 5);
         const i32 rg = tr16(mul32_q31(mul16(32767, N), celt_rcp(N + factor * K)));
         const i32 theta = tr16(mul16_q15(rg, rg) >> 1);
@@ -344,21 +352,30 @@
             stride2 = 1;
             while ((stride2 * stride2 + stride2) * B + (B >> 2) < N) stride2++;
         }
-        if (defer) {
-            defer->x = x;
-            defer->blen = blen;
-            defer->logB = logB;
-            defer->stride2 = stride2;
-            defer->c = c;
-            defer->s = s;
-            defer->on = true;
-            return cm;
-        }
+        job.x = x;
+        job.blen = blen;
+        job.logB = logB;
+        job.stride2 = stride2;
+        job.c = c;
+        job.s = s;
+        job.on = true;
+        return true;
+    }
+    return false;
+}
+OG_DEV u32 pvq_leaf_lane(i16 *xv, const PvqLds &T, int n, int k, u32 i, int pos, int B, i32 gain, int spread, RotJob *defer = nullptr) {
+    const u32 cm = pvq_leaf_walk(SpecArena{xv}, T, n, k, i, pos, B, gain);
+    OG_MARK(59);
+    if (defer) {
+        pvq_leaf_rotation(n, k, B, pos, spread, *defer);
+        return cm;
+    }
+    RotJob job;
+    if (pvq_leaf_rotation(n, k, B, pos, spread, job))
         for (int blk2 = 0; blk2 < B; blk2++) {
-            if (stride2) rotate1_lane(xv, x + blk2 * blen, blen, stride2, s, c);
-            rotate1_lane(xv, x + blk2 * blen, blen, 1, c, s);
-        }
-    }
+            if (job.stride2) rotate1_lane(xv, pos + blk2 * job.blen, job.blen, job.stride2, job.s, job.c);
+            rotate1_lane(xv, pos + blk2 * job.blen, job.blen, 1, job.c, job.s);
+        }
     return cm;
 }
 
@@ -858,12 +875,14 @@
             S.tf_res[i] = rec->tf_res[i];
         }
 #endif
-        OG_FOR_LANES(i, 2 * NBANDS) S.job_mask_row()[i] = 0;
+        if (!(rx.flags & RF_LEAVES_DONE)) {
+            OG_FOR_LANES(i, 2 * NBANDS) S.job_mask_row()[i] = 0;
 #ifdef OG_HOST_EMUL
-        OG_FOR_LANES(i, 2 * 960) S.v[V_X + i] = 0;
+            OG_FOR_LANES(i, 2 * 960) S.v[V_X + i] = 0;
 #else
-        OG_FOR_LANES(i, 2 * 960 / 8) *reinterpret_cast<og_v4i *>(&S.v[V_X + 8 * i]) = og_v4i{0, 0, 0, 0};
-#endif
+            OG_FOR_LANES(i, 2 * 960 / 8) *reinterpret_cast<og_v4i *>(&S.v[V_X + 8 * i]) = og_v4i{0, 0, 0, 0};
+#endif
+        }
     }
     return true;
 }
@@ -919,6 +938,40 @@
 #endif
 }
 
+#ifndef OG_HOST_EMUL
+OG_DEV void recon_leaves_done(const ParseRec *rec, const LeafOut *lo, const ReconCtx &rx, bool pre, u32 g0) {
+    const int n_leaves = rx.h.n_leaves, spread = (int)(rx.flags >> RF_SPREAD_SHIFT) & 3;
+    OG_MARK(2);
+    {
+        constexpr int NP = 2 * 960 / 8, NR = (NP + OG_NLANES - 1) / OG_NLANES;
+        const og_v4i *const src = reinterpret_cast<const og_v4i *>(lo->x);
+        og_v4i piece[NR];
+#pragma unroll
+        for (int r = 0; r < NR; r++) piece[r] = src[OG_MIN(OG_LANE + r * OG_NLANES, NP - 1)];
+        const u32 jm = lo->job_mask[OG_MIN(OG_LANE, 2 * NBANDS - 1)];
+#pragma unroll
+        for (int r = 0; r < NR; r++)
+            if (OG_LANE + r * OG_NLANES < NP) *reinterpret_cast<og_v4i *>(&S.v[V_X + 8 * (OG_LANE + r * OG_NLANES)]) = piece[r];
+        if (OG_LANE < 2 * NBANDS) S.job_mask_row()[OG_LANE] = jm;
+    }
+    OG_LSYNC();
+    for (int t0 = 0; t0 < n_leaves; t0 += OG_NLANES) {
+        const int t = t0 + OG_LANE;
+        RotJob job;
+        job.x = job.blen = job.logB = job.stride2 = 0;
+        job.c = job.s = 0;
+        job.on = false;
+        if (t < n_leaves) {
+            const u32 g = pre && t0 == 0 ? g0 : rec->leaf[t].geom;
+            pvq_leaf_rotation((int)(g >> 11) & 255, (int)(g >> 19) & 255, (int)(g >> 27) + 1, V_X + (int)(g & 2047), spread, job);
+        }
+        OG_MARK(28);
+        pvq_rotate_wave(S.v, job, S.rot_marker());
+    }
+    OG_LSYNC();
+}
+#endif
+
 OG_DEV int recon_result(const ReconCtx &rx) { return (rx.leaves && (rx.flags & RF_TELL_OVERFLOW)) ? INTERNAL_ERROR : rx.ret; }
 OG_DEV void recon_bookkeeping(StreamState *st, const ReconCtx &rx) {
     if (OG_LANE == 0) {
@@ -998,6 +1051,7 @@
     ReconCtx rx;
     rx.mode_after = mode_after;
     recon_hdr_load(st, rec, rx.h);
+    rx.h.flags &= ~(u32)RF_LEAVES_DONE;
     if (!recon_begin(st, rec, mode, ch, role, rx)) return rx.ret;
     if (rx.leaves) {
         pvq_tab_load();
diff --git a/esp32-opus-player_amd/csrc/og_ctx.hpp b/esp32-opus-player_amd/csrc/og_ctx.hpp
--- a/esp32-opus-player_amd/csrc/og_ctx.hpp
+++ b/esp32-opus-player_amd/csrc/og_ctx.hpp
@@ -93,6 +93,8 @@
     int host_parts = 8;
     void *d_recs[6] = {}, *d_rout[6] = {};
     size_t cap_recs[6] = {}, cap_rout[6] = {};
+    void *d_leaf_out[3] = {};
+    size_t cap_leaf_out[3] = {};
     void *d_handoff[OG_SILK_SETS] = {}, *d_srecs[OG_SILK_SETS] = {};
     size_t cap_handoff[OG_SILK_SETS] = {}, cap_srecs[OG_SILK_SETS] = {};
     const void *last_srecs = nullptr;
@@ -101,6 +103,7 @@
     int split_celt = 1;
     int split_hybrid = 1;
     int fast_recon = 1;
+    int pvq_kernel = 1;
     int mode = OPUSGPU_MODE_REFERENCE;
     int pipeline = 0;
     long long stall_ticks = 0;
diff --git a/esp32-opus-player_amd/csrc/og_debug.hpp b/esp32-opus-player_amd/csrc/og_debug.hpp
--- a/esp32-opus-player_amd/csrc/og_debug.hpp
+++ b/esp32-opus-player_amd/csrc/og_debug.hpp
@@ -3,7 +3,7 @@
 #include <string.h>
 
 struct og_debug_knobs {
-    int split = 1, split_hybrid = 1, fast_recon = 1, hybrid_recon_aside = 1, silk_params_aside = 1, silk_nb_kernel = 1, halves = 1, silk_pipeline = 1, hybrid_pipeline = 1, parse_wide = 1, parse_groups = 1, parse_priority = 1, host_parts = 16, host_slices = 1, host_timing = 0,
+    int split = 1, split_hybrid = 1, fast_recon = 1, pvq_kernel = 1, hybrid_recon_aside = 1, silk_params_aside = 1, silk_nb_kernel = 1, halves = 1, silk_pipeline = 1, hybrid_pipeline = 1, parse_wide = 1, parse_groups = 1, parse_priority = 1, host_parts = 16, host_slices = 1, host_timing = 0,
         pages_timing = 0, launch_delay_us = 0, stall_stream = 0, stall_us = 0;
 };
 inline const og_debug_knobs &og_debug() {
@@ -21,6 +21,7 @@
         flag("OPUSGPU_SPLIT", v.split);
         flag("OPUSGPU_SPLIT_HYBRID", v.split_hybrid);
         flag("OPUSGPU_FAST_RECON", v.fast_recon);
+        flag("OPUSGPU_PVQ_KERNEL", v.pvq_kernel);
         number("OPUSGPU_HYBRID_RECON_ASIDE", v.hybrid_recon_aside, 0, 2);
         flag("OPUSGPU_SILK_PARAMS_ASIDE", v.silk_params_aside);
         flag("OPUSGPU_SILK_NB_KERNEL", v.silk_nb_kernel);
diff --git a/esp32-opus-player_amd/csrc/og_pvq.hip b/esp32-opus-player_amd/csrc/og_pvq.hip
--- /dev/null
+++ b/esp32-opus-player_amd/csrc/og_pvq.hip
@@ -0,0 +1,16 @@
+#include <hip/hip_runtime.h>
+#include "og_celt_pvq.hpp"
+
+using namespace og;
+
+__global__ void __launch_bounds__(64) k_celt_pvq(const FrameDesc *__restrict__ descs, ParseRec *recs, LeafOut *lout, int n, int n_streams) {
+    __shared__ PvqBlockLds L;
+    const int f0 = (int)blockIdx.x * PVQ_BLOCK;
+    if (f0 < n) pvq_block_wave(L, descs + f0, recs + f0, lout + f0, n - f0, n_streams);
+}
+
+extern "C" void og_launch_celt_pvq(hipStream_t s, const void *descs, void *recs, void *leaf_out, int n, int n_streams) {
+    hipLaunchKernelGGL(k_celt_pvq, dim3((n + PVQ_BLOCK - 1) / PVQ_BLOCK), dim3(64), 0, s, (const FrameDesc *)descs, (ParseRec *)recs,
+                       (LeafOut *)leaf_out, n, n_streams);
+}
+extern "C" const size_t og_leaf_out_bytes = sizeof(LeafOut);
diff --git a/esp32-opus-player_amd/csrc/og_recon.hip b/esp32-opus-player_amd/csrc/og_recon.hip
--- a/esp32-opus-player_amd/csrc/og_recon.hip
+++ b/esp32-opus-player_amd/csrc/og_recon.hip
@@ -9,7 +9,7 @@
 
 __global__ void __launch_bounds__(64, OG_FAST_WAVES) k_celt_recon_fb(const FrameDesc *__restrict__ descs, StreamState *st,
                                                                            const ParseRec *recs, ReconOut *rout, int n, int n_streams,
-                                                                           int hybrid, u32 *started) {
+                                                                           int hybrid, u32 *started, const LeafOut *lout) {
     if (started && threadIdx.x == 0 && (blockIdx.x & 63) == 0) __hip_atomic_fetch_add(started, 1u, __ATOMIC_RELAXED, __HIP_MEMORY_SCOPE_SYSTEM);
     const int f = (int)blockIdx.x;
     StreamState *sp = nullptr;
@@ -44,6 +44,7 @@
             rx.pre_logE2 = sp->celt.logE2[lane < 2 * NBANDS ? lane : 0];
             rx.pre = true;
             recon_hdr_unpack(lane < 16 ? w_rec : w_st, rx.h);
+            if (!lout) rx.h.flags &= ~(u32)RF_LEAVES_DONE;
             if (mode == MODE_HYBRID && (rx.h.flags & RF_SKIP)) ok = false;
         }
         if (ok) {
@@ -57,18 +58,22 @@
         }
     }
     if (mine && rx.leaves) {
-        pvq_tab_load();
-        OG_SYNC();
-        recon_leaves_own(rec, rx, true, lg, la, li);
+        if (rx.flags & RF_LEAVES_DONE)
+            recon_leaves_done(rec, &lout[f], rx, true, lg);
+        else {
+            pvq_tab_load();
+            OG_SYNC();
+            recon_leaves_own(rec, rx, true, lg, la, li);
+        }
     }
     if (mine) recon_finish(sp, rec, rx);
     OG_PROF_FLUSH();
 }
 
 extern "C" void og_launch_celt_recon_fb(hipStream_t s, const void *descs, void *streams, const void *recs, void *rout, int n,
-                                        int n_streams, int hybrid, unsigned *started) {
+                                        int n_streams, int hybrid, unsigned *started, const void *leaf_out) {
     hipLaunchKernelGGL(k_celt_recon_fb, dim3(n), dim3(64), 0, s, (const FrameDesc *)descs, (StreamState *)streams,
-                       (const ParseRec *)recs, (ReconOut *)rout, n, n_streams, hybrid, started);
+                       (const ParseRec *)recs, (ReconOut *)rout, n, n_streams, hybrid, started, (const LeafOut *)leaf_out);
 }
 extern "C" int og_celt_recon_fb_signals(int n) { return (n + 63) / 64; }
 
diff --git a/esp32-opus-player_amd/csrc/og_step.hpp b/esp32-opus-player_amd/csrc/og_step.hpp
--- a/esp32-opus-player_amd/csrc/og_step.hpp
+++ b/esp32-opus-player_amd/csrc/og_step.hpp
@@ -45,6 +45,7 @@
     bool keeps_kind, any_silk, any_celt;
     int sset;
     void *recs, *rout, *handoff, *srecs;
+    void *leaf_out = nullptr;
 };
 
 void launch_stream_stall(opusgpu_ctx *ctx, hipStream_t q);
@@ -56,12 +57,14 @@
 void launch_celt_parse(opusgpu_ctx *ctx, hipStream_t q, const Step &st, size_t f0, int cnt, bool wide, bool early);
 int celt_parse_early_grid(const opusgpu_ctx *ctx, int cnt, bool wide);
 void launch_celt_recon_fb(opusgpu_ctx *ctx, hipStream_t q, const Step &st, size_t f0, int cnt, bool counts_in);
+void launch_celt_pvq(opusgpu_ctx *ctx, hipStream_t q, const Step &st, size_t f0, int cnt) __attribute__((weak));
 extern "C" int og_celt_recon_fb_signals(int n);
 void launch_celt_recon(opusgpu_ctx *ctx, hipStream_t q, const Step &st, size_t f0, int cnt);
 void launch_celt_post(opusgpu_ctx *ctx, hipStream_t q, const Step &st, size_t f0, int cnt, bool others);
 void launch_silk_synth(opusgpu_ctx *ctx, hipStream_t q, const Step &st, size_t f0, int cnt, int nb_done);
 void launch_silk_synth_nb(opusgpu_ctx *ctx, hipStream_t q, const Step &st, size_t f0, int cnt);
 extern const size_t og_parse_rec_bytes, og_recon_out_bytes, og_silk_handoff_bytes, og_silk_rec_bytes;
+extern "C" const size_t og_leaf_out_bytes __attribute__((weak));
 
 static int sync_in_flight(opusgpu_ctx *ctx) {
     if (ctx->sp.parse_stream) {
@@ -127,6 +130,11 @@
         return rc;
     if (ctx->cap_rout[par] < og_recon_out_bytes * need && (rc = grow(ctx, &ctx->d_rout[par], &ctx->cap_rout[par], og_recon_out_bytes * need)))
         return rc;
+    return OPUSGPU_OK;
+}
+static bool step_uses_pvq_kernel(const opusgpu_ctx *ctx) { return ctx->pvq_kernel && ctx->fast_recon && launch_celt_pvq && &og_leaf_out_bytes; }
+static int grow_leaf_out(opusgpu_ctx *ctx, int par, size_t need) {
+    if (ctx->cap_leaf_out[par] < og_leaf_out_bytes * need) return grow(ctx, &ctx->d_leaf_out[par], &ctx->cap_leaf_out[par], og_leaf_out_bytes * need);
     return OPUSGPU_OK;
 }
 
@@ -331,6 +339,10 @@
         stall(ctx, st, ctx->sp.parse_stream);
         launch_celt_parse(ctx, ctx->sp.parse_stream, st, 0, n, wide, true);
         ctx->sp.parse_started_total += (uint32_t)grid;
+    }
+    if (st.leaf_out) {
+        stall(ctx, st, ctx->sp.parse_stream);
+        launch_celt_pvq(ctx, ctx->sp.parse_stream, st, 0, n);
     }
     HIPCHK(ctx, hipEventRecord(ctx->sp.ev_parsed, ctx->sp.parse_stream));
     hipStream_t const back = ctx->sp.recon_stream;
@@ -404,6 +416,10 @@
     if (ctx->split_hybrid && st.any_silk)
         if (int rc = grow_silk_set(ctx, st.sset, (size_t)n, pipe_silk ? st.s : nullptr)) return rc;
     st.recs = ctx->d_recs[par], st.rout = ctx->d_rout[par];
+    if (pipe && step_uses_pvq_kernel(ctx)) {
+        if (int rc = grow_leaf_out(ctx, par, (size_t)n)) return rc;
+        st.leaf_out = ctx->d_leaf_out[par];
+    }
     st.handoff = ctx->split_hybrid && st.any_silk ? ctx->d_handoff[st.sset] : nullptr;
     st.srecs = ctx->split_hybrid && st.any_silk ? ctx->d_srecs[st.sset] : nullptr;
     ctx->last_recs = st.recs;
@@ -426,7 +442,11 @@
     if (ctx->pipeline && m == 4 && ctx->split_celt && ctx->mode != OPUSGPU_MODE_RFC) {
         HIPCHK(ctx, hipSetDevice(ctx->device));
         for (int par = 0; par < 3; par++)
+        {
             if (int rc = grow_step_slot(ctx, par, (size_t)max_n)) return rc;
+            if (step_uses_pvq_kernel(ctx))
+                if (int rc = grow_leaf_out(ctx, par, (size_t)max_n)) return rc;
+        }
     }
     for (int k = 0; k < n_steps; k++) {
         const int next_n = k + 1 < n_steps ? n[k + 1] : 0;
```

Result: slower. 33.29 million frames/s (-24.7%).
